# cmgcds/SParSH-AMG

Measured on AMD Instinct MI355X. Metric: AMG-PCG solve iterations/sec (7-pt 3D Poisson, fp64) + HBM GB/s (roofline: dominant kernel; config.whole_iteration: the iteration), higher is better.
Workload: dtype f64

## Files before the change

include/sparsh_amg.h:

```cpp
#ifndef SPARSH_AMG_H_
#define SPARSH_AMG_H_

#ifdef __cplusplus
extern "C" {
#endif

#define SPARSH_OK 0
#define SPARSH_EINVAL -1
#define SPARSH_ENODEV -2
#define SPARSH_ESTATE -3
#define SPARSH_ENUMERIC -4
#define SPARSH_ENOCONV -5
#define SPARSH_ECOMM -6

#define SPARSH_AMG 0
#define SPARSH_CG 1
#define SPARSH_PCG 2
#define SPARSH_BICG 3
#define SPARSH_PBICG 4
#define SPARSH_GMRES 5
#define SPARSH_PGMRES 6

#define SPARSH_SMOOTH_JACOBI 0
#define SPARSH_SMOOTH_SOR 1
#define SPARSH_SOR_FORWARD 0
#define SPARSH_SOR_SYMMETRIC 1

typedef struct sparsh_params {
    double omega;
    double tol;
    int sweeps;
    int max_levels;
    int limit_upper;
    int limit_lower;
    int coarsening;
    int max_iter;
    int coarse_limit;
    int host_threads;
    int device;
    int print_setup;
    int print_solve;
    int check_every;
    int use_graph;
    int replicate_rows;
    int precond_fp32;
    int dense_limit;
    int extend_until;
    int coarse_factor_mb;
} sparsh_params;

typedef struct sparsh_handle_s *sparsh_handle;

const char *sparsh_last_error(void);
int sparsh_version(void);
int sparsh_device_count(void);
int sparsh_host_cpus(void);

void sparsh_default_params(sparsh_params *p);

int sparsh_create_csr(int nrow, int ncol, const int *rowptr, const int *colindex, const double *val, sparsh_handle *out);
void sparsh_destroy(sparsh_handle h);

int sparsh_setup(sparsh_handle h, const sparsh_params *p);

int sparsh_set_stopping(sparsh_handle h, double tol, int max_iter, int check_every);

int sparsh_set_kernel_config(sparsh_handle h, int kind, int vec, int nt, int remap);

int sparsh_level_format(sparsh_handle h, int level, int *kind, long *stored_entries);

int sparsh_level_layout(sparsh_handle h, int level, long *slots, long *value_blocks, long *meta_bytes);
int sparsh_set_const_slots(sparsh_handle h, int enable);
int sparsh_set_index_compression(sparsh_handle h, int mode);
int sparsh_set_alternate_sweeps(sparsh_handle h, int mode);
int sparsh_set_paired_restriction(sparsh_handle h, int enable);
int sparsh_set_fused_prolongation(sparsh_handle h, int enable);
int sparsh_set_constant_diagonal(sparsh_handle h, int enable);
int sparsh_set_double_sweep(sparsh_handle h, int mode);
int sparsh_set_marching_ops(sparsh_handle h, int mode);
int sparsh_set_zero_start(sparsh_handle h, int enable);
int sparsh_set_deferred_x(sparsh_handle h, int enable);
int sparsh_level_marching_ops(sparsh_handle h, int level, int *on, int *plan, double *table_us, double *marching_us);
int sparsh_set_box_plan(sparsh_handle h, int level, int kernel, int q, int ty, int cz);
int sparsh_level_double_sweep(sparsh_handle h, int level, int *on, int *dims, int *plan, double *single_us, double *double_us);
int sparsh_level_constant_diagonal(sparsh_handle h, int level, int *is_const, double *value);
int sparsh_level_prolong_fused(sparsh_handle h, int level, int *fused);
int sparsh_level_paired(sparsh_handle h, int level, int *paired);
int sparsh_set_fused_zero_sweep(sparsh_handle h, int mode);
int sparsh_set_placement_search(sparsh_handle h, int enable);
int sparsh_placement_info(sparsh_handle h, double *chosen_us, double *worst_us, double *initial_us, int *triples, double *seconds);
int sparsh_set_setup_broadcast(sparsh_handle h, int enable);
int sparsh_setup_share_info(sparsh_handle h, int *built_locally, long *image_bytes);
long sparsh_debug_hierarchy_roundtrip(sparsh_handle h, long truncate_to);
int sparsh_level_index16(sparsh_handle h, int level, long *blocks16, long *blocks);
int sparsh_debug_index16_roundtrip(int nrow, const int *rowptr, const int *colindex, long *blocks16, long *blocks);
int sparsh_set_tile(sparsh_handle h, int enable);
int sparsh_level_tile_rows(sparsh_handle h, int level, int *rows);
int sparsh_bench_comm(sparsh_handle h, int what, int level, int reps, double *avg_seconds);
const char *sparsh_level_kernel(sparsh_handle h, int level);
int sparsh_level_placement(sparsh_handle h, int level, int *nt, int *remap);

int sparsh_setup_host(sparsh_handle h, const sparsh_params *p);

int sparsh_num_levels(sparsh_handle h);
int sparsh_level_info(sparsh_handle h, int level, int *nrow, int *nnz, int *p_ncol, int *p_nnz);
int sparsh_level_csr(sparsh_handle h, int level, int which, int *rowptr, int *colindex, double *val);
int sparsh_coarse_inverse(sparsh_handle h, double *inv);
int sparsh_coarse_info(sparsh_handle h, int *info6, long *bytes);
int sparsh_set_coarse_form(sparsh_handle h, int form, int leaf, int merge_rows);
int sparsh_set_coarse_top_merge(sparsh_handle h, int top_merge_rows);
int sparsh_coarse_nd_info(sparsh_handle h, int *info6);
int sparsh_coarse_window(sparsh_handle h, int *window);
int sparsh_set_coarse_interface(sparsh_handle h, int enable);
int sparsh_set_coarse_block(sparsh_handle h, int rows);
double sparsh_setup_seconds(sparsh_handle h);

int sparsh_vcycle(sparsh_handle h, const double *b, double *x, int iterations, double *hist, int hist_cap, int *ncycles);

int sparsh_vcycle_dev(sparsh_handle h, const double *b_dev, double *x_dev, int iterations, double *hist, int hist_cap, int *ncycles);

int sparsh_solve(sparsh_handle h, int method, const double *b, double *x, double *hist, int hist_cap, int *iters);

int sparsh_solve_dev(sparsh_handle h, int method, const double *b_dev, double *x_dev, int max_iters, double *hist, int hist_cap, int *iters, double *seconds);

int sparsh_krylov_init_dev(sparsh_handle h, int method, const double *b_dev, double *x_dev);
int sparsh_krylov_step_dev(sparsh_handle h, int nsteps, int *done, double *residual);
int sparsh_krylov_history(sparsh_handle h, double *hist, int hist_cap, int *iters);

int sparsh_op_spmv(sparsh_handle h, int level, const double *x, double *y);
int sparsh_op_jacobi(sparsh_handle h, int level, const double *b, double *x, int sweeps, int x_is_zero);
int sparsh_op_residual(sparsh_handle h, int level, const double *b, const double *x, double *r);
int sparsh_op_resnorm(sparsh_handle h, int level, const double *b, const double *x, double *nrm);
int sparsh_op_restrict(sparsh_handle h, int level, const double *r, double *bc);
int sparsh_op_residual_restrict(sparsh_handle h, int level, const double *b, const double *x, double *bc, double *xc);
int sparsh_op_prolong(sparsh_handle h, int level, const double *xc, double *xf);
int sparsh_op_jacobi_prolong(sparsh_handle h, int level, const double *b, const double *x, double *xf);
int sparsh_op_spmv_dot(sparsh_handle h, int level, const double *x, double *y, double *dot);
int sparsh_op_jacobi_dot(sparsh_handle h, int level, const double *b, const double *x, double *y, double *dot);
int sparsh_op_coarse(sparsh_handle h, const double *b, double *x);
int sparsh_op_precond_f32(sparsh_handle h, const double *r, double *z);
int sparsh_op_precond(sparsh_handle h, const double *r, double *z);
int sparsh_op_dot(sparsh_handle h, int n, const double *x, const double *y, double *out);
int sparsh_op_nrm2(sparsh_handle h, int n, const double *x, double *out);
int sparsh_op_axpby(sparsh_handle h, int n, double a, const double *x, double bcoef, double *y);

int sparsh_bench_op(sparsh_handle h, int op, int level, int reps, double *avg_seconds);

#define SPARSH_BASIS_FP64 0
#define SPARSH_BASIS_FP32 1
int sparsh_set_gmres(sparsh_handle h, int restart);
int sparsh_gmres_info(sparsh_handle h, int *restart, long *basis_bytes);
int sparsh_set_gmres_basis(sparsh_handle h, int precision);
int sparsh_gmres_basis(sparsh_handle h, int *precision);

int sparsh_set_smoother(sparsh_handle h, int kind, int sweeps, int order);
int sparsh_level_colors(sparsh_handle h, int level, int *ncolors, int *rows_per_color);
int sparsh_level_color_of_rows(sparsh_handle h, int level, int *color);
int sparsh_op_sor(sparsh_handle h, int level, const double *b, double *x, int sweeps, int reverse, int x_is_zero);
int sparsh_set_sor_path(sparsh_handle h, int mode);
int sparsh_level_sor_layout(sparsh_handle h, int level, int *ncolors, int *single_launch, long *bytes);

int sparsh_dev_alloc(sparsh_handle h, long nbytes, void **out);
int sparsh_dev_free(sparsh_handle h, void *p);
int sparsh_dev_fill(sparsh_handle h, double *dst_dev, long n, double value);
int sparsh_h2d(sparsh_handle h, void *dst_dev, const void *src, long nbytes);
int sparsh_d2h(sparsh_handle h, void *dst, const void *src_dev, long nbytes);
// ... 40 lines not shown
```

sparsh_amg_amd/__init__.py:

```python
from __future__ import annotations

import ctypes as C
import os

import numpy as np

from . import problems

_HERE = os.path.dirname(os.path.abspath(__file__))
LIB_PATH = os.path.join(_HERE, "libsparsh_amg.so")

SPARSH_AMG, SPARSH_CG, SPARSH_PCG, SPARSH_BICG, SPARSH_PBICG = 0, 1, 2, 3, 4
SPARSH_GMRES, SPARSH_PGMRES = 5, 6
METHODS = {"amg": SPARSH_AMG, "cg": SPARSH_CG, "pcg": SPARSH_PCG, "bicg": SPARSH_BICG, "pbicg": SPARSH_PBICG,
           "gmres": SPARSH_GMRES, "pgmres": SPARSH_PGMRES}
SPARSH_SMOOTH_JACOBI, SPARSH_SMOOTH_SOR = 0, 1
SPARSH_SOR_FORWARD, SPARSH_SOR_SYMMETRIC = 0, 1
SPARSH_BASIS_FP64, SPARSH_BASIS_FP32 = 0, 1
GMRES_BASES = {"fp64": SPARSH_BASIS_FP64, "fp32": SPARSH_BASIS_FP32}
SMOOTHERS = {"jacobi": SPARSH_SMOOTH_JACOBI, "sor": SPARSH_SMOOTH_SOR}
SOR_ORDERS = {"forward": SPARSH_SOR_FORWARD, "symmetric": SPARSH_SOR_SYMMETRIC}
SPARSH_OK, SPARSH_EINVAL, SPARSH_ENODEV, SPARSH_ESTATE, SPARSH_ENUMERIC, SPARSH_ENOCONV, SPARSH_ECOMM = 0, -1, -2, -3, -4, -5, -6

c_int_p = C.POINTER(C.c_int)
c_dbl_p = C.POINTER(C.c_double)


class SparshError(RuntimeError):
    def __init__(self, code, msg):
        super().__init__(f"sparsh error {code}: {msg}")
        self.code = code


class Params(C.Structure):

    _fields_ = [
        ("omega", C.c_double),
        ("tol", C.c_double),
        ("sweeps", C.c_int),
        ("max_levels", C.c_int),
        ("limit_upper", C.c_int),
        ("limit_lower", C.c_int),
        ("coarsening", C.c_int),
        ("max_iter", C.c_int),
        ("coarse_limit", C.c_int),
        ("host_threads", C.c_int),
        ("device", C.c_int),
        ("print_setup", C.c_int),
        ("print_solve", C.c_int),
        ("check_every", C.c_int),
        ("use_graph", C.c_int),
        ("replicate_rows", C.c_int),
        ("precond_fp32", C.c_int),
        ("dense_limit", C.c_int),
        ("extend_until", C.c_int),
        ("coarse_factor_mb", C.c_int),
    ]


def _load():
    if not os.path.exists(LIB_PATH):
        raise ImportError(
            f"{LIB_PATH} is missing: build it with `python -c 'import __graft_entry__ as g; g.build()'` "
            "(or `make -C sparsh_amg_amd/csrc`).  There is no pure-Python/CPU fallback."
        )
    L = C.CDLL(LIB_PATH)
    H = C.c_void_p
    P = C.POINTER
    sig = {
        "sparsh_last_error": (C.c_char_p, []),
        "sparsh_version": (C.c_int, []),
        "sparsh_device_count": (C.c_int, []),
        "sparsh_host_cpus": (C.c_int, []),
        "sparsh_default_params": (None, [P(Params)]),
        "sparsh_create_csr": (C.c_int, [C.c_int, C.c_int, c_int_p, c_int_p, c_dbl_p, P(H)]),
        "sparsh_destroy": (None, [H]),
        "sparsh_setup": (C.c_int, [H, P(Params)]),
        "sparsh_setup_host": (C.c_int, [H, P(Params)]),
        "sparsh_set_stopping": (C.c_int, [H, C.c_double, C.c_int, C.c_int]),
        "sparsh_set_kernel_config": (C.c_int, [H, C.c_int, C.c_int, C.c_int, C.c_int]),
        "sparsh_level_placement": (C.c_int, [H, C.c_int, c_int_p, c_int_p]),
        "sparsh_level_format": (C.c_int, [H, C.c_int, c_int_p, C.POINTER(C.c_long)]),
        "sparsh_level_layout": (C.c_int, [H, C.c_int, C.POINTER(C.c_long), C.POINTER(C.c_long), C.POINTER(C.c_long)]),
        "sparsh_set_const_slots": (C.c_int, [H, C.c_int]),
        "sparsh_set_tile": (C.c_int, [H, C.c_int]),
        "sparsh_set_index_compression": (C.c_int, [H, C.c_int]),
        "sparsh_set_alternate_sweeps": (C.c_int, [H, C.c_int]),
        "sparsh_set_paired_restriction": (C.c_int, [H, C.c_int]),
        "sparsh_set_fused_prolongation": (C.c_int, [H, C.c_int]),
        "sparsh_set_constant_diagonal": (C.c_int, [H, C.c_int]),
        "sparsh_set_double_sweep": (C.c_int, [H, C.c_int]),
        "sparsh_set_marching_ops": (C.c_int, [H, C.c_int]),
        "sparsh_set_zero_start": (C.c_int, [H, C.c_int]),
        "sparsh_set_deferred_x": (C.c_int, [H, C.c_int]),
        "sparsh_level_marching_ops": (C.c_int, [H, C.c_int, C.POINTER(C.c_int), C.POINTER(C.c_int), C.POINTER(C.c_double), C.POINTER(C.c_double)]),
        "sparsh_level_double_sweep": (C.c_int, [H, C.c_int, C.POINTER(C.c_int), C.POINTER(C.c_int), C.POINTER(C.c_int), C.POINTER(C.c_double),
                                                  C.POINTER(C.c_double)]),
        "sparsh_level_constant_diagonal": (C.c_int, [H, C.c_int, C.POINTER(C.c_int), C.POINTER(C.c_double)]),
        "sparsh_level_prolong_fused": (C.c_int, [H, C.c_int, C.POINTER(C.c_int)]),
        "sparsh_op_jacobi_prolong": (C.c_int, [H, C.c_int, c_dbl_p, c_dbl_p, c_dbl_p]),
        "sparsh_set_box_plan": (C.c_int, [H, C.c_int, C.c_int, C.c_int, C.c_int, C.c_int]),
        "sparsh_op_spmv_dot": (C.c_int, [H, C.c_int, c_dbl_p, c_dbl_p, c_dbl_p]),
        "sparsh_op_jacobi_dot": (C.c_int, [H, C.c_int, c_dbl_p, c_dbl_p, c_dbl_p, c_dbl_p]),
        "sparsh_level_paired": (C.c_int, [H, C.c_int, C.POINTER(C.c_int)]),
        "sparsh_set_fused_zero_sweep": (C.c_int, [H, C.c_int]),
        "sparsh_set_placement_search": (C.c_int, [H, C.c_int]),
        "sparsh_placement_info": (C.c_int, [H, C.POINTER(C.c_double), C.POINTER(C.c_double), C.POINTER(C.c_double), c_int_p, C.POINTER(C.c_double)]),
        "sparsh_debug_index16_roundtrip": (C.c_int, [C.c_int, c_int_p, c_int_p, C.POINTER(C.c_long), C.POINTER(C.c_long)]),
        "sparsh_set_setup_broadcast": (C.c_int, [H, C.c_int]),
        "sparsh_debug_hierarchy_roundtrip": (C.c_long, [H, C.c_long]),
        "sparsh_setup_share_info": (C.c_int, [H, C.POINTER(C.c_int), C.POINTER(C.c_long)]),
        "sparsh_level_index16": (C.c_int, [H, C.c_int, C.POINTER(C.c_long), C.POINTER(C.c_long)]),
        "sparsh_level_tile_rows": (C.c_int, [H, C.c_int, c_int_p]),
        "sparsh_bench_comm": (C.c_int, [H, C.c_int, C.c_int, C.c_int, c_dbl_p]),
        "sparsh_level_kernel": (C.c_char_p, [H, C.c_int]),
        "sparsh_num_levels": (C.c_int, [H]),
        "sparsh_level_info": (C.c_int, [H, C.c_int, c_int_p, c_int_p, c_int_p, c_int_p]),
        "sparsh_level_csr": (C.c_int, [H, C.c_int, C.c_int, c_int_p, c_int_p, c_dbl_p]),
        "sparsh_coarse_inverse": (C.c_int, [H, c_dbl_p]),
        "sparsh_op_precond_f32": (C.c_int, [H, c_dbl_p, c_dbl_p]),
        "sparsh_coarse_info": (C.c_int, [H, c_int_p, C.POINTER(C.c_long)]),
        "sparsh_coarse_window": (C.c_int, [H, c_int_p]),
        "sparsh_set_coarse_interface": (C.c_int, [H, C.c_int]),
        "sparsh_set_coarse_block": (C.c_int, [H, C.c_int]),
        "sparsh_set_coarse_form": (C.c_int, [H, C.c_int, C.c_int, C.c_int]),
        "sparsh_coarse_nd_info": (C.c_int, [H, c_int_p]),
        "sparsh_set_coarse_top_merge": (C.c_int, [H, C.c_int]),
        "sparsh_setup_seconds": (C.c_double, [H]),
        "sparsh_vcycle": (C.c_int, [H, c_dbl_p, c_dbl_p, C.c_int, c_dbl_p, C.c_int, c_int_p]),
        "sparsh_vcycle_dev": (C.c_int, [H, C.c_void_p, C.c_void_p, C.c_int, c_dbl_p, C.c_int, c_int_p]),
        "sparsh_solve": (C.c_int, [H, C.c_int, c_dbl_p, c_dbl_p, c_dbl_p, C.c_int, c_int_p]),
        "sparsh_solve_dev": (C.c_int, [H, C.c_int, C.c_void_p, C.c_void_p, C.c_int, c_dbl_p, C.c_int, c_int_p, c_dbl_p]),
        "sparsh_set_device": (C.c_int, [C.c_int]),
        "sparsh_comm_unique_id": (C.c_int, [C.c_char_p]),
        "sparsh_comm_init_rccl": (C.c_int, [H, C.c_char_p, C.c_int, C.c_int]),
        "sparsh_local_range": (C.c_int, [H, C.c_int, c_int_p, c_int_p, c_int_p]),
        "sparsh_set_overlap": (C.c_int, [H, C.c_int]),
        "sparsh_comm_group_create": (C.c_int, [C.c_int, P(C.c_void_p)]),
        "sparsh_comm_group_destroy": (None, [C.c_void_p]),
        "sparsh_set_deep_halo": (C.c_int, [H, C.c_int]),
        "sparsh_dist_deep_op": (C.c_int, [H, C.c_int, C.c_int, C.c_int, C.c_int, C.c_int, c_int_p]),
        "sparsh_dist_deep_op_get": (C.c_int, [H, c_int_p, c_int_p, c_dbl_p, c_int_p, c_int_p, c_int_p, c_int_p, c_int_p, c_int_p]),
        "sparsh_deep_info": (C.c_int, [H, C.c_int, c_int_p]),
        "sparsh_deep_layer_end": (C.c_int, [H, C.c_int, C.c_int, c_int_p]),
        "sparsh_deep_prefix_spmv": (C.c_int, [H, C.c_int, C.c_int, c_dbl_p, c_dbl_p]),
        "sparsh_exchanges_issued": (C.c_long, [H]),
        "sparsh_comm_group_fail_after": (C.c_int, [C.c_void_p, C.c_int]),
        "sparsh_comm_group_set_delay": (C.c_int, [C.c_void_p, C.c_double]),
        "sparsh_set_comm_tuning": (C.c_int, [H, C.c_int]),
        "sparsh_comm_schedule": (C.c_int, [H, C.c_int, c_int_p, c_dbl_p]),
        "sparsh_comm_measured": (C.c_int, [H, c_dbl_p]),
        "sparsh_plan_comm_schedule": (C.c_int, [H, C.c_int, c_dbl_p]),
        "sparsh_comm_init_group": (C.c_int, [H, C.c_void_p, C.c_int]),
        "sparsh_dist_local_op": (C.c_int, [H, C.c_int, C.c_int, C.c_int, C.c_int, c_int_p]),
        "sparsh_dist_local_op_get": (C.c_int, [H, c_int_p, c_int_p, c_dbl_p, c_int_p, c_int_p, c_int_p, c_int_p]),
        "sparsh_krylov_init_dev": (C.c_int, [H, C.c_int, C.c_void_p, C.c_void_p]),
        "sparsh_krylov_step_dev": (C.c_int, [H, C.c_int, c_int_p, c_dbl_p]),
        "sparsh_krylov_history": (C.c_int, [H, c_dbl_p, C.c_int, c_int_p]),
        "sparsh_op_spmv": (C.c_int, [H, C.c_int, c_dbl_p, c_dbl_p]),
        "sparsh_op_jacobi": (C.c_int, [H, C.c_int, c_dbl_p, c_dbl_p, C.c_int, C.c_int]),
        "sparsh_op_residual": (C.c_int, [H, C.c_int, c_dbl_p, c_dbl_p, c_dbl_p]),
        "sparsh_op_resnorm": (C.c_int, [H, C.c_int, c_dbl_p, c_dbl_p, c_dbl_p]),
        "sparsh_op_restrict": (C.c_int, [H, C.c_int, c_dbl_p, c_dbl_p]),
        "sparsh_op_residual_restrict": (C.c_int, [H, C.c_int, c_dbl_p, c_dbl_p, c_dbl_p, c_dbl_p]),
        "sparsh_op_prolong": (C.c_int, [H, C.c_int, c_dbl_p, c_dbl_p]),
        "sparsh_op_coarse": (C.c_int, [H, c_dbl_p, c_dbl_p]),
        "sparsh_op_dot": (C.c_int, [H, C.c_int, c_dbl_p, c_dbl_p, c_dbl_p]),
        "sparsh_op_nrm2": (C.c_int, [H, C.c_int, c_dbl_p, c_dbl_p]),
        "sparsh_op_axpby": (C.c_int, [H, C.c_int, C.c_double, c_dbl_p, C.c_double, c_dbl_p]),
        "sparsh_bench_op": (C.c_int, [H, C.c_int, C.c_int, C.c_int, c_dbl_p]),
        "sparsh_dev_alloc": (C.c_int, [H, C.c_long, P(C.c_void_p)]),
        "sparsh_dev_free": (C.c_int, [H, C.c_void_p]),
        "sparsh_dev_fill": (C.c_int, [H, C.c_void_p, C.c_long, C.c_double]),
        "sparsh_h2d": (C.c_int, [H, C.c_void_p, C.c_void_p, C.c_long]),
        "sparsh_d2h": (C.c_int, [H, C.c_void_p, C.c_void_p, C.c_long]),
        "sparsh_sync": (C.c_int, [H]),
        "sparsh_profile": (C.c_int, [H, C.c_int]),
        "sparsh_set_smoother": (C.c_int, [H, C.c_int, C.c_int, C.c_int]),
        "sparsh_level_colors": (C.c_int, [H, C.c_int, c_int_p, c_int_p]),
        "sparsh_level_color_of_rows": (C.c_int, [H, C.c_int, c_int_p]),
        "sparsh_op_sor": (C.c_int, [H, C.c_int, c_dbl_p, c_dbl_p, C.c_int, C.c_int, C.c_int]),
        "sparsh_set_sor_path": (C.c_int, [H, C.c_int]),
        "sparsh_level_sor_layout": (C.c_int, [H, C.c_int, c_int_p, c_int_p, C.POINTER(C.c_long)]),
        "sparsh_profile_read": (C.c_int, [H, c_dbl_p]),
        "sparsh_set_gmres": (C.c_int, [H, C.c_int]),
        "sparsh_gmres_info": (C.c_int, [H, c_int_p, C.POINTER(C.c_long)]),
        "sparsh_set_gmres_basis": (C.c_int, [H, C.c_int]),
        "sparsh_gmres_basis": (C.c_int, [H, c_int_p]),
        "sparsh_op_precond": (C.c_int, [H, c_dbl_p, c_dbl_p]),
    }
    for name, (res, args) in sig.items():
        fn = getattr(L, name)
        fn.restype = res
        fn.argtypes = args
    return L


lib = _load()


def _dp(a):
    return a.ctypes.data_as(c_dbl_p)


def _ip(a):
    return a.ctypes.data_as(c_int_p)


def _check(rc, allow=()):
    if rc != SPARSH_OK and rc not in allow:
        raise SparshError(rc, lib.sparsh_last_error().decode())
    return rc


def default_params(**kw) -> Params:
    p = Params()
    lib.sparsh_default_params(C.byref(p))
    for k, v in kw.items():
        if not hasattr(p, k):
            raise AttributeError(f"sparsh_params has no field {k}")
        setattr(p, k, v)
    return p


def set_device(device: int):
    _check(lib.sparsh_set_device(device))


def comm_unique_id() -> bytes:
    buf = C.create_string_buffer(128)
    _check(lib.sparsh_comm_unique_id(buf))
    return buf.raw


def comm_group_create(nranks: int):
    g = C.c_void_p()
    _check(lib.sparsh_comm_group_create(nranks, C.byref(g)))
    return g


def comm_group_destroy(g):
    lib.sparsh_comm_group_destroy(g)


def comm_group_set_delay(g, microseconds: float):
    _check(lib.sparsh_comm_group_set_delay(g, float(microseconds)))


def comm_group_fail_after(g, ncalls: int):
    _check(lib.sparsh_comm_group_fail_after(g, int(ncalls)))


def index16_roundtrip(rowptr, colindex):
    rp = np.ascontiguousarray(rowptr, dtype=np.int32)
    ci = np.ascontiguousarray(colindex, dtype=np.int32)
    a, b = C.c_long(), C.c_long()
    _check(lib.sparsh_debug_index16_roundtrip(len(rp) - 1, _ip(rp), _ip(ci), C.byref(a), C.byref(b)))
    return a.value, b.value


def device_count() -> int:
    return lib.sparsh_device_count()


def host_cpus() -> int:
    return lib.sparsh_host_cpus()


class sp_matrix_mg:

    def __init__(self, rowptr, colindex, val, ncol=None):
        self.rowptr = np.ascontiguousarray(rowptr, dtype=np.int32)
        self.colindex = np.ascontiguousarray(colindex, dtype=np.int32)
        self.val = np.ascontiguousarray(val, dtype=np.float64)
        self.nrow = len(self.rowptr) - 1
        self.ncol = self.nrow if ncol is None else int(ncol)
        self.nnz = int(self.rowptr[-1])
        if len(self.colindex) < self.nnz or len(self.val) < self.nnz:
            raise ValueError("colindex/val shorter than rowptr[-1]")
        h = C.c_void_p()
        _check(lib.sparsh_create_csr(self.nrow, self.ncol, _ip(self.rowptr), _ip(self.colindex), _dp(self.val), C.byref(h)))
        self._h = h
        self.params = None

    def close(self):
        if getattr(self, "_h", None):
            lib.sparsh_destroy(self._h)
            self._h = None

    def __del__(self):
        try:
            self.close()
        except Exception:
            pass

    def set_const_slots(self, enable=True):
        _check(lib.sparsh_set_const_slots(self._h, int(bool(enable))))
        return self

    def set_setup_broadcast(self, enable=True):
        _check(lib.sparsh_set_setup_broadcast(self._h, int(bool(enable))))
        return self

    def hierarchy_roundtrip(self, truncate_to=-1):
        r = lib.sparsh_debug_hierarchy_roundtrip(self._h, int(truncate_to))
        if r < 0:
            _check(int(r))
        return int(r)

    def setup_share_info(self):
        a, b = C.c_int(), C.c_long()
        _check(lib.sparsh_setup_share_info(self._h, C.byref(a), C.byref(b)))
        return bool(a.value), b.value

    def set_placement_search(self, enable=True):
        _check(lib.sparsh_set_placement_search(self._h, int(bool(enable))))
        return self

    def placement_info(self):
        a, b, c, k, t = C.c_double(), C.c_double(), C.c_double(), C.c_int(), C.c_double()
        _check(lib.sparsh_placement_info(self._h, C.byref(a), C.byref(b), C.byref(c), C.byref(k), C.byref(t)))
        return {"chosen_us": round(a.value, 2), "worst_us": round(b.value, 2), "initial_us": round(c.value, 2), "triples": k.value,
                "seconds": round(t.value, 3)}

    def set_fused_zero_sweep(self, enable=2):
        _check(lib.sparsh_set_fused_zero_sweep(self._h, int(enable)))
        return self

    def set_alternate_sweeps(self, mode=1):
        _check(lib.sparsh_set_alternate_sweeps(self._h, int(mode)))
        return self

    def set_double_sweep(self, mode=1):
        _check(lib.sparsh_set_double_sweep(self._h, int(mode)))
        return self

    def level_double_sweep(self, level):
        on = C.c_int(0)
        dims, plan = (C.c_int * 3)(), (C.c_int * 3)()
        t1, t2 = C.c_double(0.0), C.c_double(0.0)
        _check(lib.sparsh_level_double_sweep(self._h, int(level), C.byref(on), dims, plan, C.byref(t1), C.byref(t2)))
        return {"on": bool(on.value), "grid": list(dims), "points_per_thread": plan[0], "lines_per_tile": plan[1], "planes_per_chunk": plan[2],
                "two_single_sweeps_us": round(t1.value, 2), "double_sweep_us": round(t2.value, 2)}

    def set_deferred_x(self, enable=True):
        _check(lib.sparsh_set_deferred_x(self._h, 1 if enable else 0))
        return self

    def set_zero_start(self, enable=True):
        _check(lib.sparsh_set_zero_start(self._h, 1 if enable else 0))
        return self

    def set_marching_ops(self, mode=1):
        _check(lib.sparsh_set_marching_ops(self._h, int(mode)))
        return self

    def level_marching_ops(self, level):
        on = C.c_int(0)
        plan = (C.c_int * 3)()
        t1, t2 = C.c_double(0.0), C.c_double(0.0)
        _check(lib.sparsh_level_marching_ops(self._h, int(level), C.byref(on), plan, C.byref(t1), C.byref(t2)))
        return {"on": bool(on.value), "points_per_thread": plan[0], "lines_per_tile": plan[1], "planes_per_chunk": plan[2],
                "table_kernel_us": round(t1.value, 2), "marching_kernel_us": round(t2.value, 2)}

    def set_box_plan(self, level, kernel, q=0, ty=0, cz=0, shared_cu=False):
        k = {"double": 2, "marching": 1}.get(kernel, kernel)
        if shared_cu:
            if k != 1:
                raise ValueError("shared_cu is a plan of the marching kernel")
            k = 3
        _check(lib.sparsh_set_box_plan(self._h, int(level), int(k), int(q), int(ty), int(cz)))
        return self

    def set_constant_diagonal(self, enable=True):
        _check(lib.sparsh_set_constant_diagonal(self._h, 1 if enable else 0))
        return self

    def level_constant_diagonal(self, level):
        f, v = C.c_int(0), C.c_double(0.0)
        _check(lib.sparsh_level_constant_diagonal(self._h, int(level), C.byref(f), C.byref(v)))
        return bool(f.value), v.value

    def set_fused_prolongation(self, enable=True):
        _check(lib.sparsh_set_fused_prolongation(self._h, 1 if enable else 0))
        return self

    def level_prolong_fused(self, level):
        v = C.c_int(0)
        _check(lib.sparsh_level_prolong_fused(self._h, int(level), C.byref(v)))
        return v.value

    def op_jacobi_prolong(self, level, b, x, xf):
        b = np.ascontiguousarray(b, dtype=np.float64)
        x = np.ascontiguousarray(x, dtype=np.float64)
        xf = np.array(xf, dtype=np.float64)
        _check(lib.sparsh_op_jacobi_prolong(self._h, int(level), _dp(b), _dp(x), _dp(xf)))
        return xf

    def set_paired_restriction(self, enable=True):
        _check(lib.sparsh_set_paired_restriction(self._h, 1 if enable else 0))
        return self

    def level_paired(self, level):
        v = C.c_int(0)
        _check(lib.sparsh_level_paired(self._h, int(level), C.byref(v)))
        return v.value

    def set_index_compression(self, mode=1):
        _check(lib.sparsh_set_index_compression(self._h, int(mode)))
        return self

    def level_index16(self, level):
        a, b = C.c_long(), C.c_long()
        _check(lib.sparsh_level_index16(self._h, level, C.byref(a), C.byref(b)))
        return a.value, b.value

    def set_tile(self, enable=True):
        _check(lib.sparsh_set_tile(self._h, int(bool(enable))))
        return self

    def level_tile_rows(self, level):
        r = C.c_int(0)
        _check(lib.sparsh_level_tile_rows(self._h, level, C.byref(r)))
        return r.value

    def set_smoother(self, kind="jacobi", sweeps=0, order="forward"):
        k = SMOOTHERS[kind] if isinstance(kind, str) else int(kind)
        o = SOR_ORDERS[order] if isinstance(order, str) else int(order)
        _check(lib.sparsh_set_smoother(self._h, k, int(sweeps), o))
        return self

    def set_gmres(self, restart=0, basis=None):
        _check(lib.sparsh_set_gmres(self._h, int(restart)))
        if basis is not None:
            _check(lib.sparsh_set_gmres_basis(self._h, GMRES_BASES[basis] if isinstance(basis, str) else int(basis)))
        return self

    def gmres_basis(self):
        p = C.c_int()
        _check(lib.sparsh_gmres_basis(self._h, C.byref(p)))
        return {v: k for k, v in GMRES_BASES.items()}[p.value]

    def gmres_info(self):
        m, nbytes = C.c_int(), C.c_long()
        _check(lib.sparsh_gmres_info(self._h, C.byref(m), C.byref(nbytes)))
        info = dict(restart=m.value, basis_bytes=nbytes.value)
        if self.gmres_basis() != "fp64":
            info["basis"] = self.gmres_basis()
        return info

    def level_colors(self, level):
        nc = C.c_int(0)
        _check(lib.sparsh_level_colors(self._h, level, C.byref(nc), None))
        counts = np.zeros(max(nc.value, 1), dtype=np.int32)
        _check(lib.sparsh_level_colors(self._h, level, C.byref(nc), _ip(counts)))
# ... 215 lines not shown
        _check(lib.sparsh_dist_deep_op_get(self._h, _ip(rp), _ip(ci), _dp(v), _ip(gof), _ip(le), _ip(si), _ip(ss), _ip(rpos), _ip(rs)))
        M = sp.csr_matrix((v[:nnz], ci[:nnz], rp), shape=(nrow, nall))
        recv = rs[: 3 * nrs].reshape(-1, 3)
        nrecv = int(recv[:, 2].sum()) if len(recv) else 0
        plan = dict(nloc=nloc, npad=npad, nall=nall, global_of=gof[:nall], layer_end=le, send_idx=si[:nsend],
                    send=ss[: 3 * nss].reshape(-1, 3), recv=recv, recv_pos=rpos[:nrecv])
        return M, plan

    def vcycle(self, b, x, iterations=-1, hist_cap=8192):
        b = np.ascontiguousarray(b, dtype=np.float64)
        hist = np.zeros(hist_cap)
        n = C.c_int()
        rc = _check(lib.sparsh_vcycle(self._h, _dp(b), _dp(x), iterations, _dp(hist), hist_cap, C.byref(n)), allow=(SPARSH_ENOCONV,))
        return hist[: min(n.value, hist_cap)].copy(), rc

    def solve(self, method, b, x, hist_cap=8192, allow=()):
        b = np.ascontiguousarray(b, dtype=np.float64)
        assert x.dtype == np.float64 and x.flags.c_contiguous
        hist = np.zeros(hist_cap)
        n = C.c_int()
        m = METHODS[method] if isinstance(method, str) else method
        rc = _check(lib.sparsh_solve(self._h, m, _dp(b), _dp(x), _dp(hist), hist_cap, C.byref(n)), allow=(SPARSH_ENOCONV,) + tuple(allow))
        return hist[: min(n.value, hist_cap)].copy(), rc

    def dev_alloc(self, nbytes):
        p = C.c_void_p()
        _check(lib.sparsh_dev_alloc(self._h, nbytes, C.byref(p)))
        return p

    def dev_free(self, p):
        _check(lib.sparsh_dev_free(self._h, p))

    def dev_fill(self, dptr, n, value=0.0):
        _check(lib.sparsh_dev_fill(self._h, dptr, n, value))

    def h2d(self, dptr, arr):
        arr = np.ascontiguousarray(arr)
        _check(lib.sparsh_h2d(self._h, dptr, arr.ctypes.data_as(C.c_void_p), arr.nbytes))

    def d2h(self, arr, dptr):
        _check(lib.sparsh_d2h(self._h, arr.ctypes.data_as(C.c_void_p), dptr, arr.nbytes))

    def sync(self):
        _check(lib.sparsh_sync(self._h))

    def solve_dev(self, method, b_dev, x_dev, max_iters=0, hist_cap=8192):
        hist = np.zeros(hist_cap)
        n = C.c_int()
        sec = C.c_double()
        m = METHODS[method] if isinstance(method, str) else method
        rc = _check(
            lib.sparsh_solve_dev(self._h, m, b_dev, x_dev, max_iters, _dp(hist), hist_cap, C.byref(n), C.byref(sec)),
            allow=(SPARSH_ENOCONV,),
        )
        return hist[: min(n.value, hist_cap)].copy(), n.value, sec.value, rc

    def krylov_init_dev(self, method, b_dev, x_dev):
        m = METHODS[method] if isinstance(method, str) else method
        _check(lib.sparsh_krylov_init_dev(self._h, m, b_dev, x_dev))

    def krylov_step_dev(self, nsteps):
        done = C.c_int()
        res = C.c_double()
        _check(lib.sparsh_krylov_step_dev(self._h, nsteps, C.byref(done), C.byref(res)))
        return done.value, res.value

    def krylov_history(self, hist_cap=8192):
        hist = np.zeros(hist_cap)
        n = C.c_int()
        _check(lib.sparsh_krylov_history(self._h, _dp(hist), hist_cap, C.byref(n)))
        return hist[: min(n.value, hist_cap)].copy()

    def profile(self, enable=True):
        _check(lib.sparsh_profile(self._h, 1 if enable else 0))

    def profile_read(self):
        out = np.zeros(4)
        _check(lib.sparsh_profile_read(self._h, _dp(out)))
        return dict(launches=int(out[0]), seconds=out[1], nrow=int(out[2]), nnz=int(out[3]))

    def bench_op(self, op, level=0, reps=20):
        ops = {"spmv": 0, "jacobi": 1, "residual": 2, "restrict": 3, "prolong": 4, "coarse": 5, "dot": 6, "axpby": 7, "copy_int": 8,
               "jacobi_pingpong": 9, "jacobi_pingpong_resident": 10, "jacobi_double": 11, "sor": 12,
               "gmres_orth": 13, "gmres_orth_unfused": 14, "gmres_orth_fp32_basis": 15}
        sec = C.c_double()
        _check(lib.sparsh_bench_op(self._h, ops[op] if isinstance(op, str) else op, level, reps, C.byref(sec)))
        return sec.value

    def op_spmv(self, level, x):
        x = np.ascontiguousarray(x, dtype=np.float64)
        y = np.zeros(self.level_info(level)["nrow"])
        _check(lib.sparsh_op_spmv(self._h, level, _dp(x), _dp(y)))
        return y

    def op_jacobi(self, level, b, x, sweeps, x_is_zero=False):
        b = np.ascontiguousarray(b, dtype=np.float64)
        x = np.array(x, dtype=np.float64)
        _check(lib.sparsh_op_jacobi(self._h, level, _dp(b), _dp(x), sweeps, 1 if x_is_zero else 0))
        return x

    def op_sor(self, level, b, x, sweeps, reverse=False, x_is_zero=False):
        b = np.ascontiguousarray(b, dtype=np.float64)
        x = np.array(x, dtype=np.float64)
        _check(lib.sparsh_op_sor(self._h, level, _dp(b), _dp(x), int(sweeps), 1 if reverse else 0, 1 if x_is_zero else 0))
        return x

    def op_residual(self, level, b, x):
        b = np.ascontiguousarray(b, dtype=np.float64)
        x = np.ascontiguousarray(x, dtype=np.float64)
        r = np.zeros_like(b)
        _check(lib.sparsh_op_residual(self._h, level, _dp(b), _dp(x), _dp(r)))
        return r

    def op_resnorm(self, level, b, x):
        b = np.ascontiguousarray(b, dtype=np.float64)
        x = np.ascontiguousarray(x, dtype=np.float64)
        out = C.c_double()
        _check(lib.sparsh_op_resnorm(self._h, level, _dp(b), _dp(x), C.byref(out)))
        return out.value

    def op_spmv_dot(self, level, x):
        x = np.ascontiguousarray(x, dtype=np.float64)
        y = np.zeros(self.level_info(level)["nrow"])
        dot = C.c_double()
        _check(lib.sparsh_op_spmv_dot(self._h, int(level), _dp(x), _dp(y), C.byref(dot)))
        return y, dot.value

    def op_jacobi_dot(self, level, b, x):
        b = np.ascontiguousarray(b, dtype=np.float64)
        x = np.ascontiguousarray(x, dtype=np.float64)
        y = np.zeros_like(b)
        dot = C.c_double()
        _check(lib.sparsh_op_jacobi_dot(self._h, int(level), _dp(b), _dp(x), _dp(y), C.byref(dot)))
        return y, dot.value

    def op_restrict(self, level, r):
        r = np.ascontiguousarray(r, dtype=np.float64)
        bc = np.zeros(self.level_info(level + 1)["nrow"])
        _check(lib.sparsh_op_restrict(self._h, level, _dp(r), _dp(bc)))
        return bc

    def op_residual_restrict(self, level, b, x):
        b = np.ascontiguousarray(b, dtype=np.float64)
        x = np.ascontiguousarray(x, dtype=np.float64)
        nc = self.level_info(level + 1)["nrow"]
        bc, xc = np.zeros(nc), np.zeros(nc)
        _check(lib.sparsh_op_residual_restrict(self._h, level, _dp(b), _dp(x), _dp(bc), _dp(xc)))
        return bc, xc

    def op_prolong(self, level, xc, xf):
        xc = np.ascontiguousarray(xc, dtype=np.float64)
        xf = np.array(xf, dtype=np.float64)
        _check(lib.sparsh_op_prolong(self._h, level, _dp(xc), _dp(xf)))
        return xf

    def op_coarse(self, b):
        b = np.ascontiguousarray(b, dtype=np.float64)
        x = np.zeros_like(b)
        _check(lib.sparsh_op_coarse(self._h, _dp(b), _dp(x)))
        return x

    def op_precond_f32(self, r):
        r = np.ascontiguousarray(r, dtype=np.float64)
        z = np.zeros_like(r)
        _check(lib.sparsh_op_precond_f32(self._h, _dp(r), _dp(z)))
        return z

# ... 65 lines not shown
```

sparsh_amg_amd/csrc/capi.cpp:

```cpp
#include <algorithm>
#include <cmath>
#include <cstdio>
#include <cstdlib>
#include <cstring>
#include <memory>
#include <string>
#include <vector>

#include <hip/hip_runtime_api.h>

#include "../../include/sparsh_amg.h"
#include "engine.hpp"

using namespace sparsh;

struct sparsh_handle_s {
    std::unique_ptr<Engine> eng;
    LocalOp cached_op;
    DeepLocal cached_deep;
};

namespace {

thread_local std::string g_err;
// ... 370 lines not shown
    return SPARSH_OK;
}

int sparsh_set_alternate_sweeps(sparsh_handle h, int enable)
{
    if (!h || !h->eng) return fail(SPARSH_EINVAL, "null handle");
    if (enable < 0 || enable > 2) return fail(SPARSH_EINVAL, "mode must be 0 (never), 1 (where a sweep streams more than the Infinity Cache holds) or 2 (always)");
    h->eng->kernel_cfg().alt_dir = enable;
    h->eng->config_changed();
    return SPARSH_OK;
}

int sparsh_set_double_sweep(sparsh_handle h, int mode)
{
    if (!h || !h->eng) return fail(SPARSH_EINVAL, "null handle");
    if (mode < 0 || mode > 2) return fail(SPARSH_EINVAL, "mode must be 0 (never), 1 (where the setup measures it faster) or 2 (wherever the level is a box grid with a plan)");
    h->eng->kernel_cfg().box2 = mode;
    h->eng->config_changed();
    return SPARSH_OK;
}

int sparsh_level_double_sweep(sparsh_handle h, int level, int *on, int *dims, int *plan, double *single_us, double *double_us)
{
    REQUIRE_READY(h);
    REQUIRE_LEVEL(h, level);
    const DevLevel &L = h->eng->level(level);
    if (on) *on = (!h->eng->distributed() || L.replicated) && box2_applies(L.A, h->eng->kernel_cfg()) ? 1 : 0;
    if (dims) {
        dims[0] = L.A.box_nx;
        dims[1] = L.A.box_ny;
        dims[2] = L.A.box_nz;
    }
    if (plan) {
        plan[0] = L.A.box_q;
        plan[1] = L.A.box_ty;
        plan[2] = L.A.box_cz;
    }
    if (single_us) *single_us = L.box_single_us;
    if (double_us) *double_us = L.box_double_us;
    return SPARSH_OK;
}

int sparsh_set_deferred_x(sparsh_handle h, int enable)
{
    if (!h || !h->eng) return fail(SPARSH_EINVAL, "null handle");
    h->eng->kernel_cfg().defer_x = enable != 0;
    h->eng->config_changed();
    return SPARSH_OK;
}

int sparsh_set_zero_start(sparsh_handle h, int enable)
{
    if (!h || !h->eng) return fail(SPARSH_EINVAL, "null handle");
    h->eng->kernel_cfg().zero_start = enable != 0;
    h->eng->config_changed();
    return SPARSH_OK;
}

int sparsh_set_marching_ops(sparsh_handle h, int mode)
{
    if (!h || !h->eng) return fail(SPARSH_EINVAL, "null handle");
    if (mode < 0 || mode > 2) return fail(SPARSH_EINVAL, "mode must be 0 (never), 1 (where the setup measures it faster) or 2 (wherever the level is a box grid with a plan)");
    h->eng->kernel_cfg().box1 = mode;
    h->eng->config_changed();
    return SPARSH_OK;
}

int sparsh_level_marching_ops(sparsh_handle h, int level, int *on, int *plan, double *table_us, double *marching_us)
{
    REQUIRE_READY(h);
    REQUIRE_LEVEL(h, level);
    const DevLevel &L = h->eng->level(level);
    if (on) *on = (!h->eng->distributed() || L.replicated) && box1_applies(L.A, h->eng->kernel_cfg()) ? 1 : 0;
    if (plan) {
        plan[0] = L.A.box1_q;
        plan[1] = L.A.box1_ty;
        plan[2] = L.A.box1_cz;
    }
    if (table_us) *table_us = L.box1_table_us;
    if (marching_us) *marching_us = L.box1_us;
    return SPARSH_OK;
}

int sparsh_set_box_plan(sparsh_handle h, int level, int kernel, int q, int ty, int cz)
{
    REQUIRE_READY(h);
    REQUIRE_LEVEL(h, level);
    const int rc = h->eng->set_box_plan(level, kernel, q, ty, cz);
    return rc == SPARSH_OK ? SPARSH_OK : fail(rc, h->eng->error);
}

int sparsh_set_constant_diagonal(sparsh_handle h, int enable)
{
    if (!h || !h->eng) return fail(SPARSH_EINVAL, "null handle");
    h->eng->kernel_cfg().const_diag = enable != 0;
    h->eng->config_changed();
    return SPARSH_OK;
}

int sparsh_level_constant_diagonal(sparsh_handle h, int level, int *is_const, double *value)
{
    REQUIRE_READY(h);
    REQUIRE_LEVEL(h, level);
    const DevLevel &L = h->eng->level(level);
    if (is_const) *is_const = h->eng->diag_stream(L) == nullptr ? 1 : 0;
    if (value) *value = L.diag_const;
    return SPARSH_OK;
}

int sparsh_set_fused_prolongation(sparsh_handle h, int enable)
{
    if (!h || !h->eng) return fail(SPARSH_EINVAL, "null handle");
    h->eng->kernel_cfg().fuse_prolong = enable != 0;
    h->eng->config_changed();
    return SPARSH_OK;
}

int sparsh_level_prolong_fused(sparsh_handle h, int level, int *fused)
{
    REQUIRE_READY(h);
    REQUIRE_LEVEL(h, level);
    if (!fused) return fail(SPARSH_EINVAL, "null output");
    *fused = !h->eng->level_prolong_fused(level) ? 0 : (h->eng->level(level - 1).pair_aggregates ? 1 : 2);
    return SPARSH_OK;
}

int sparsh_set_paired_restriction(sparsh_handle h, int enable)
{
    if (!h || !h->eng) return fail(SPARSH_EINVAL, "null handle");
    h->eng->kernel_cfg().pair_restrict = enable != 0;
    h->eng->config_changed();
    return SPARSH_OK;
}

int sparsh_level_paired(sparsh_handle h, int level, int *paired)
{
    REQUIRE_READY(h);
    REQUIRE_LEVEL(h, level);
    if (!paired) return fail(SPARSH_EINVAL, "null output");
    *paired = h->eng->level_paired(level);
    return SPARSH_OK;
}

int sparsh_set_index_compression(sparsh_handle h, int mode)
{
    if (!h || !h->eng) return fail(SPARSH_EINVAL, "null handle");
    if (mode < 0 || mode > 2) return fail(SPARSH_EINVAL, "mode must be 0 (off), 1 (operators that stream from HBM through the CSR-stream kernel) or 2 (every operator)");
    h->eng->kernel_cfg().idx16 = mode;
    h->eng->config_changed();
    return SPARSH_OK;
}

int sparsh_level_index16(sparsh_handle h, int level, long *blocks16, long *blocks)
{
    REQUIRE_READY(h);
    REQUIRE_LEVEL(h, level);
    const DevCsr &A = h->eng->level(level).A;
    if (blocks16) *blocks16 = A.col16 ? A.nblk16 : 0;
    if (blocks) *blocks = A.nblk;
    return SPARSH_OK;
}

int sparsh_set_smoother(sparsh_handle h, int kind, int sweeps, int order)
{
    if (!h || !h->eng) return fail(SPARSH_EINVAL, "null handle");
    Engine &E = *h->eng;
    if (kind != SPARSH_SMOOTH_JACOBI && kind != SPARSH_SMOOTH_SOR)
        return fail(SPARSH_EINVAL, "kind must be SPARSH_SMOOTH_JACOBI (0) or SPARSH_SMOOTH_SOR (1)");
    if (sweeps < 0) return fail(SPARSH_EINVAL, "sweeps < 0");
    if (order != SPARSH_SOR_FORWARD && order != SPARSH_SOR_SYMMETRIC)
        return fail(SPARSH_EINVAL, "order must be SPARSH_SOR_FORWARD (0) or SPARSH_SOR_SYMMETRIC (1)");
    if (kind == SPARSH_SMOOTH_JACOBI && sweeps > 0 && E.ready() && E.distributed())
// ... 744 lines not shown
}

int sparsh_op_nrm2(sparsh_handle h, int n, const double *x, double *out)
{
    double d = 0.0;
    int rc = sparsh_op_dot(h, n, x, x, &d);
    if (rc == SPARSH_OK) *out = std::sqrt(d);
    return rc;
}

int sparsh_op_axpby(sparsh_handle h, int n, double a, const double *x, double bcoef, double *y)
{
    REQUIRE_READY(h);
    REQUIRE_SINGLE(h);
    if (n <= 0) return fail(SPARSH_EINVAL, "n <= 0");
    Engine &E = *h->eng;
    DBuf dx(E, (size_t)n, x), dy(E, (size_t)n, y);
    launch_axpby(n, a, dx.p, bcoef, dy.p, E.stream());
    return done(E, dy.get(y));
}

int sparsh_bench_op(sparsh_handle h, int op, int level, int reps, double *avg_seconds)
{
    REQUIRE_READY(h);
    REQUIRE_LEVEL(h, level);
    if (reps <= 0 || !avg_seconds) return fail(SPARSH_EINVAL, "bad reps");
    Engine &E = *h->eng;
    const DevLevel &L = E.level(level);
    const size_t n = (size_t)L.n;
    const bool has_coarse = level + 1 < E.nlevels();
    if ((op == 3 || op == 4) && !has_coarse) return fail(SPARSH_EINVAL, "no coarser level");
    const size_t nc = has_coarse ? (size_t)E.level(level + 1).n : 1;
    const size_t xh = (size_t)std::max(L.planA.nhalo, L.planR.nhalo), ch = (size_t)L.planP.nhalo;
    DBuf x(E, n + xh), y(E, n), b(E, n), c(E, nc + ch);
    std::vector<double> ones(std::max(n, nc), 1.0);
    (void)hipMemcpy(x.p, ones.data(), n * 8, hipMemcpyHostToDevice);
    (void)hipMemcpy(b.p, ones.data(), n * 8, hipMemcpyHostToDevice);
    (void)hipMemcpy(y.p, ones.data(), n * 8, hipMemcpyHostToDevice);
    (void)hipMemcpy(c.p, ones.data(), nc * 8, hipMemcpyHostToDevice);
    hipStream_t st = E.stream();
    auto run = [&]() {
        switch (op) {
        case 0: E.op_spmv(level, x.p, y.p); break;
        case 1: {
            CsrArgs a;
            a.x = x.p;
            a.b = b.p;
            a.d = L.diag;
            a.y = y.p;
            a.omega = E.params().omega;
            launch_csr(L.A, OP_JACOBI, a, L.fine, st, E.kernel_cfg());
        } break;
        case 2: E.op_residual(level, b.p, x.p, y.p); break;
        case 3: E.op_restrict(level, x.p, c.p); break;
        case 4: E.op_prolong(level, c.p, y.p); break;
        case 5: E.op_coarse(E.level(E.nlevels() - 1).b ? E.level(E.nlevels() - 1).b : b.p, E.level(E.nlevels() - 1).r); break;
        case 6: {
            int nb = 0;
            launch_dot((int)n, x.p, b.p, E.level(0).r, &nb, st);
        } break;
        case 7: launch_axpby((int)n, 0.5, x.p, 0.5, y.p, st); break;
        case 8: launch_copy_int((int)n, L.A.rowptr, reinterpret_cast<int *>(y.p), st); break;
        case 9:
        case 10: {
            static thread_local int flip = 0;
            double *xa = op == 9 ? x.p : L.x, *xb = op == 9 ? y.p : L.x2;
            CsrArgs a;
            a.x = (flip & 1) ? xb : xa;
            a.y = (flip & 1) ? xa : xb;
            a.b = op == 9 ? b.p : L.r;
            a.d = L.diag;
            a.omega = E.params().omega;
            a.reverse = csr_alternates(L.A, E.kernel_cfg()) && (flip & 1);
            ++flip;
            launch_csr(L.A, OP_JACOBI, a, L.fine, st, E.kernel_cfg());
        } break;
        case 12: E.sor_leg(level, L.r, L.x, 1, false); break;
        case 11: {
            static thread_local int flip2 = 0;
            double *xa = (flip2 & 1) ? L.x2 : L.x, *xb = (flip2 & 1) ? L.x : L.x2;
            ++flip2;
            launch_box2(L.A, xa, L.r, xb, E.params().omega, L.fine, st);
        } break;
        case 13: E.gmres_bench_step(true); break;
        case 14: E.gmres_bench_step(false); break;
        case 15: E.gmres_bench_step(true); break;
        default: break;
        }
    };
    if (op < 0 || op > 15) return fail(SPARSH_EINVAL, "unknown op");
    if (op == 13 || op == 14 || op == 15) {
        if (level != 0 || E.distributed()) return fail(SPARSH_EINVAL, "the GMRES orthogonalisation step runs on level 0 of a single-GPU handle");
        if ((op == 15) != (E.gmres_basis() == SPARSH_BASIS_FP32))
            return fail(SPARSH_ESTATE, "ops 13 and 14 run on a double basis, op 15 on a float basis (sparsh_set_gmres_basis)");
        if (int rc = E.gmres_bench_prepare(); rc != SPARSH_OK) return fail(rc, E.error);
    }
    if (op == 12 && (E.distributed() || !E.build_sor_level(level))) return fail(SPARSH_ESTATE, "no SOR layout on this handle");
    if (op == 11 && (E.distributed() || !box2_applies(L.A, E.kernel_cfg()))) return fail(SPARSH_ESTATE, "the level does not run double sweeps (sparsh_level_double_sweep)");
    for (int i = 0; i < 3; ++i) run();
    hipEvent_t e0, e1;
    (void)hipEventCreate(&e0);
    (void)hipEventCreate(&e1);
    (void)hipEventRecord(e0, st);
    for (int i = 0; i < reps; ++i) run();
    (void)hipEventRecord(e1, st);
    (void)hipEventSynchronize(e1);
    float ms = 0.f;
    (void)hipEventElapsedTime(&ms, e0, e1);
    (void)hipEventDestroy(e0);
    (void)hipEventDestroy(e1);
    *avg_seconds = ms * 1e-3 / reps;
    return SPARSH_OK;
}

int sparsh_dev_alloc(sparsh_handle h, long nbytes, void **out)
{
    if (!h || !h->eng || !out || nbytes < 0) return fail(SPARSH_EINVAL, "bad arguments");
    *out = h->eng->dalloc((size_t)nbytes);
    return *out ? SPARSH_OK : fail(SPARSH_ENODEV, h->eng->error);
}

int sparsh_dev_free(sparsh_handle h, void *p)
{
    if (!h || !h->eng) return fail(SPARSH_EINVAL, "null handle");
    h->eng->dfree(p);
    return SPARSH_OK;
}

int sparsh_dev_fill(sparsh_handle h, double *dst_dev, long n, double value)
{
    if (!h || !h->eng || !h->eng->stream()) return fail(SPARSH_EINVAL, "null handle or no stream (call sparsh_setup first)");
    if (n < 0 || n > 0x7fffffffL) return fail(SPARSH_EINVAL, "bad length");
    launch_fill((int)n, value, dst_dev, h->eng->stream());
    return SPARSH_OK;
}

int sparsh_h2d(sparsh_handle h, void *dst_dev, const void *src, long nbytes)
{
    if (!h || !h->eng) return fail(SPARSH_EINVAL, "null handle");
    if (hipMemcpy(dst_dev, src, (size_t)nbytes, hipMemcpyHostToDevice) != hipSuccess) return fail(SPARSH_ENODEV, "H2D failed");
    return SPARSH_OK;
}

int sparsh_d2h(sparsh_handle h, void *dst, const void *src_dev, long nbytes)
{
    if (!h || !h->eng) return fail(SPARSH_EINVAL, "null handle");
    if (h->eng->stream()) (void)hipStreamSynchronize(h->eng->stream());
    if (hipMemcpy(dst, src_dev, (size_t)nbytes, hipMemcpyDeviceToHost) != hipSuccess) return fail(SPARSH_ENODEV, "D2H failed");
    return SPARSH_OK;
}

int sparsh_sync(sparsh_handle h)
{
    if (!h || !h->eng) return fail(SPARSH_EINVAL, "null handle");
    if (h->eng->stream() && hipStreamSynchronize(h->eng->stream()) != hipSuccess) return fail(SPARSH_ENODEV, "sync failed");
    return SPARSH_OK;
}

int sparsh_profile(sparsh_handle h, int enable)
{
    if (!h || !h->eng) return fail(SPARSH_EINVAL, "null handle");
    if (enable) {
        h->eng->profile_begin();
        h->eng->prof.enabled = true;
    } else if (h->eng->prof.enabled) {
        h->eng->profile_collect();
        h->eng->prof.enabled = false;
    }
    return SPARSH_OK;
}

int sparsh_profile_read(sparsh_handle h, double *out4)
{
    REQUIRE_READY(h);
    out4[0] = h->eng->prof.launches;
    out4[1] = h->eng->prof.seconds;
    out4[2] = h->eng->level(0).n;
    out4[3] = h->eng->level(0).A.nnz;
    return SPARSH_OK;
}

}
```

sparsh_amg_amd/csrc/engine.cpp:

```cpp
#include "engine.hpp"

#include <algorithm>
#include <functional>
#include <cmath>
#include <cstdio>
#include <cstdlib>
#include <cstring>
#include <omp.h>

namespace sparsh {

namespace {
constexpr int kProfEvents = 8192;
}

bool Engine::check(hipError_t e, const char *what)
{
    if (e == hipSuccess) return true;
    error = std::string(what) + ": " + hipGetErrorString(e);
    return false;
}

bool Engine::note_hip(hipError_t e, const char *what)
{
// ... 485 lines not shown
    const double t0 = omp_get_wtime();
    omp_set_num_threads(p.host_threads > 0 ? p.host_threads : effective_cpus());
    std::vector<char> image;
    int rc0 = SPARSH_OK;
    std::string err0;
    if (me == 0) {
        rc0 = setup_host(p);
        err0 = error;
        if (rc0 == SPARSH_OK) serialize_hierarchy(H_, image);
    }
    built_locally_ = (me == 0);
    long long *hdr = nullptr;
    if (!check(hipMalloc(reinterpret_cast<void **>(&hdr), 16), "hipMalloc")) return SPARSH_ENODEV;
    long long h2[2] = {(long long)image.size(), (long long)rc0};
    bool good = check(hipMemcpyAsync(hdr, h2, 16, hipMemcpyHostToDevice, st_), "hipMemcpy");
    good = good && comm_->bcast(hdr, 16, 0, st_);
    good = good && check(hipMemcpyAsync(h2, hdr, 16, hipMemcpyDeviceToHost, st_), "hipMemcpy") && check(hipStreamSynchronize(st_), "hipStreamSynchronize");
    (void)hipFree(hdr);
    if (!good) {
        if (error.empty()) error = "broadcast of the hierarchy header failed: " + comm_->error;
        return SPARSH_ECOMM;
    }
    if (h2[1] != SPARSH_OK) {
        error = me == 0 ? err0 : "the setup on rank 0 failed";
        host_ready_ = false;
        return (int)h2[1];
    }
    const size_t total = (size_t)h2[0];
    image_bytes_ = total;
    if (me != 0) image.resize(total);
    const size_t chunk = std::min<size_t>(total, (size_t)256 << 20);
    char *stage = nullptr;
    {
        const bool mine = chunk == 0 || hipMalloc(reinterpret_cast<void **>(&stage), chunk) == hipSuccess;
        double *flag = nullptr;
        if (!check(hipMalloc(reinterpret_cast<void **>(&flag), sizeof(double)), "hipMalloc")) {
            if (stage) (void)hipFree(stage);
            return SPARSH_ENODEV;
        }
        double f = mine ? 0.0 : 1.0;
        bool okf = check(hipMemcpyAsync(flag, &f, sizeof(double), hipMemcpyHostToDevice, st_), "hipMemcpy") && comm_->allreduce_sum(flag, 1, st_) &&
                   check(hipMemcpyAsync(&f, flag, sizeof(double), hipMemcpyDeviceToHost, st_), "hipMemcpy") && check(hipStreamSynchronize(st_), "hipStreamSynchronize");
        (void)hipFree(flag);
        if (!okf || f != 0.0) {
            if (stage) (void)hipFree(stage);
            if (!okf) {
                if (error.empty()) error = "agreement on the hierarchy staging buffers failed: " + comm_->error;
                return SPARSH_ECOMM;
            }
            error = mine ? "another rank could not allocate its staging buffer for the hierarchy broadcast"
                         : "hipMalloc of the " + std::to_string(chunk >> 20) + " MB staging buffer for the hierarchy broadcast failed";
            return SPARSH_ENODEV;
        }
    }
    for (size_t off = 0; good && off < total; off += chunk) {
        const size_t nb = std::min(chunk, total - off);
        if (me == 0) good = check(hipMemcpyAsync(stage, image.data() + off, nb, hipMemcpyHostToDevice, st_), "hipMemcpy");
        good = good && comm_->bcast(stage, nb, 0, st_);
        if (good && me != 0) good = check(hipMemcpyAsync(image.data() + off, stage, nb, hipMemcpyDeviceToHost, st_), "hipMemcpy");
        good = good && check(hipStreamSynchronize(st_), "hipStreamSynchronize");
    }
    if (stage) (void)hipFree(stage);
    if (!good) {
        if (error.empty()) error = "broadcast of the hierarchy failed: " + comm_->error;
        return SPARSH_ECOMM;
    }
    if (me != 0) {
        prm_ = p;
        ready_ = false;
        if (!deserialize_hierarchy(image.data(), image.size(), A0_, H_)) {
            error = H_.error;
            host_ready_ = false;
            return SPARSH_ENUMERIC;
        }
        host_ready_ = true;
        setup_seconds = omp_get_wtime() - t0;
        H_.seconds = setup_seconds;
    }
    return SPARSH_OK;
}

void Engine::tune_box_kernels()
{
    for (size_t l = 0; l + 1 < lev_.size(); ++l) {
        DevLevel &L = lev_[l];
        L.A.box_on = L.A.box1_on = false;
        L.box_single_us = L.box_double_us = L.box1_table_us = L.box1_us = 0.0;
        if (L.A.box_q <= 0 || (dist_ && !L.replicated) || L.deep || csr_family(L.A, cfg_) != FAM_SDIA_TAB) continue;
        if (cfg_.box2 >= 2) L.A.box_on = true;
        if (cfg_.box1 >= 2) L.A.box1_on = L.A.box1_q > 0;
        const bool time2 = cfg_.box2 == 1, time1 = cfg_.box1 == 1 && L.A.box1_q > 0;
        if (!(time1 || time2)) continue;
        if (L.n < 400000) continue;
        hipEvent_t e0 = nullptr, e1 = nullptr;
        if (hipEventCreate(&e0) != hipSuccess || hipEventCreate(&e1) != hipSuccess) continue;
        CsrArgs a;
        a.b = L.r;
        launch_fill(L.n, 1.0, L.r, st_);
        a.d = L.diag;
        a.omega = prm_.omega;
        auto timed = [&](bool fused) -> double {
            double *p = L.x, *q = L.x2;
            const int launches = fused ? 5 : 10;
            for (int it = 0; it < launches; ++it) {
                if (it == (fused ? 1 : 2)) (void)hipEventRecord(e0, st_);
                if (fused) {
                    launch_box2(L.A, p, a.b, q, prm_.omega, L.fine, st_);
                } else {
                    a.x = p;
                    a.y = q;
                    launch_csr(L.A, OP_JACOBI, a, L.fine, st_, cfg_);
                }
                std::swap(p, q);
            }
            (void)hipEventRecord(e1, st_);
            if (hipEventSynchronize(e1) != hipSuccess) return 1e30;
            float ms = 0.f;
            (void)hipEventElapsedTime(&ms, e0, e1);
            return (double)ms * 1e3 / 4.0;
        };
        if (time2) {
            L.box_single_us = timed(false);
            L.box_double_us = timed(true);
            L.A.box_on = L.box_double_us < 0.97 * L.box_single_us;
        }
        if (time1) {
            auto timed1 = [&](bool marching) -> double {
                double *p = L.x, *q = L.x2;
                for (int it = 0; it < 8; ++it) {
                    if (it == 2) (void)hipEventRecord(e0, st_);
                    a.x = p;
                    a.y = q;
                    a.partial = part0_;
                    if (marching) launch_box1(L.A, 1, a, L.fine, st_);
                    else launch_csr(L.A, OP_JACOBI_DOT, a, L.fine, st_, cfg_);
                    std::swap(p, q);
                }
                (void)hipEventRecord(e1, st_);
                if (hipEventSynchronize(e1) != hipSuccess) return 1e30;
                float ms = 0.f;
                (void)hipEventElapsedTime(&ms, e0, e1);
                return (double)ms * 1e3 / 6.0;
            };
            L.box1_table_us = timed1(false);
            L.box1_us = timed1(true);
            {
                const int q0 = L.A.box1_q, ty0 = L.A.box1_ty, cz0 = L.A.box1_cz;
                if (box1_plan(L.A, true) && (L.A.box1_q != q0 || L.A.box1_ty != ty0 || L.A.box1_cz != cz0) && box1_workgroups(L.A) <= part_cap_) {
                    const double t_alt = timed1(true);
                    if (t_alt < L.box1_us) {
                        L.box1_us = t_alt;
                    } else {
                        L.A.box1_q = q0;
                        L.A.box1_ty = ty0;
                        L.A.box1_cz = cz0;
                    }
                } else {
                    L.A.box1_q = q0;
                    L.A.box1_ty = ty0;
                    L.A.box1_cz = cz0;
                }
            }
            L.A.box1_on = L.box1_us < 0.97 * L.box1_table_us;
        }
        (void)hipMemsetAsync(L.x, 0, (size_t)L.n * 8, st_);
        (void)hipMemsetAsync(L.x2, 0, (size_t)L.n * 8, st_);
        (void)hipMemsetAsync(L.r, 0, (size_t)L.n * 8, st_);
        (void)hipEventDestroy(e0);
        (void)hipEventDestroy(e1);
    }
}

void Engine::tune_placement()
{
    if (lev_.size() < 2) return;
    DevLevel &L = lev_[0];
    const size_t bytes = (size_t)L.n * 24;
    if (bytes < ((size_t)96 << 20) || bytes > ((size_t)512 << 20)) return;
    const CsrFamily fam = csr_family(L.A, cfg_);
    if (fam != FAM_SDIA_TAB) return;
    std::vector<double **> slots = {&L.x, &L.x2, &work_[0], &L.r};
    for (size_t k = 1; k < work_.size(); ++k) slots.push_back(&work_[k]);
    std::vector<double *> buf;
    for (double **s : slots) buf.push_back(*s);
    const size_t owned = buf.size();
    const size_t vbytes = (size_t)L.n * 8;
    for (int q = 0; q < 5; ++q) {
        void *sp = nullptr;
        if (hipMalloc(&sp, vbytes) != hipSuccess) break;
        buf.push_back(static_cast<double *>(sp));
    }
    hipEvent_t e0 = nullptr, e1 = nullptr;
    if (hipEventCreate(&e0) != hipSuccess || hipEventCreate(&e1) != hipSuccess) {
        for (size_t q = owned; q < buf.size(); ++q) (void)hipFree(buf[q]);
        return;
    }
    auto probe = [&](double *x, double *x2, double *b) -> double {
        CsrArgs a;
        a.b = b;
        a.d = L.diag;
        a.omega = prm_.omega;
        double *p = x, *q = x2;
        const bool pairs = box2_applies(L.A, cfg_);
        for (int it = 0; it < (pairs ? 5 : 10); ++it) {
            if (it == (pairs ? 1 : 2)) (void)hipEventRecord(e0, st_);
            if (pairs) {
                launch_box2(L.A, p, b, q, prm_.omega, L.fine, st_);
            } else {
                a.x = p;
                a.y = q;
                launch_csr(L.A, OP_JACOBI, a, L.fine, st_, cfg_);
            }
            std::swap(p, q);
        }
        (void)hipEventRecord(e1, st_);
        if (hipEventSynchronize(e1) != hipSuccess) return 1e30;
        float ms = 0.f;
        (void)hipEventElapsedTime(&ms, e0, e1);
        return (double)ms * 1e3 / 8.0;
    };
    const double t_begin = omp_get_wtime();
    for (double *q : buf) launch_fill(L.n, 1.0, q, st_);
    const double good_us = (double)L.n * 24.0 / 5.8e12 * 1e6 * 1.04 * (box2_applies(L.A, cfg_) ? 0.6 : 1.0);
    double best = 1e30, worst = 0.0;
    int bi = 0, bj = 1, bk = 2;
    const int nb = (int)buf.size();
    bool done = false;
    for (int hi = 2; hi < nb && !done; ++hi)
        for (int j = 1; j < hi && !done; ++j)
            for (int i = 0; i < j && !done; ++i) {
                const double t = probe(buf[i], buf[j], buf[hi]);
                if (place_tried == 0) place_first_us = t;
                ++place_tried;
                if (t < best) {
                    best = t;
                    bi = i;
                    bj = j;
                    bk = hi;
                }
                worst = std::max(worst, t);
                done = best <= good_us || place_tried >= 260;
            }
    (void)hipEventDestroy(e0);
    (void)hipEventDestroy(e1);
// ... 480 lines not shown
            const Partition &rrows = parts_[l + 1].replicated ? gather_part_ : parts_[l + 1];
            LocalOp lr = extract_local(h.R, rrows, pl, me);
            if (!upload_csr(*this, lp.M, d.P, false) || !upload_plan(lp.plan, d.planP)) return SPARSH_ENODEV;
            if (!upload_csr(*this, lr.M, d.R, false) || !upload_plan(lr.plan, d.planR)) return SPARSH_ENODEV;
            d.P_is_aggregation = h.P_is_aggregation;
            int xh = d.planA.nhalo;
            if (l > 0 && !lev_[l - 1].replicated) xh = std::max(xh, lev_[l - 1].planP.nhalo);
            xcap = (size_t)d.n + xh;
            rcap = (size_t)d.n + d.planR.nhalo;
            if (d.deep) {
                xcap = (size_t)d.layer_end[d.K];
                rcap = std::max((size_t)d.npad, (size_t)d.n + d.planR.nhalo) + 64;
                d.xc_stage = static_cast<double *>(dalloc(((size_t)d.planP.nloc + d.planP.nhalo + 64) * 8));
                if (!d.xc_stage) return SPARSH_ENODEV;
                if (l == 0) {
                    d.b_ext = static_cast<double *>(dalloc(xcap * 8));
                    if (!d.b_ext || !check(hipMemsetAsync(d.b_ext, 0, xcap * 8, st_), "hipMemsetAsync")) return SPARSH_ENODEV;
                }
            }
        }
        d.x = static_cast<double *>(dalloc(xcap * 8));
        d.x2 = static_cast<double *>(dalloc(xcap * 8));
        d.r = static_cast<double *>(dalloc(rcap * 8));
        if (l > 0) {
            const size_t bcap = d.deep ? xcap : (size_t)d.n;
            d.b = static_cast<double *>(dalloc(bcap * 8));
            if (d.b && !check(hipMemsetAsync(d.b, 0, bcap * 8, st_), "hipMemsetAsync")) return SPARSH_ENODEV;
        }
        if (!d.diag || !d.x || !d.x2 || !d.r || (l > 0 && !d.b)) return SPARSH_ENODEV;
        if (l + 1 < nl) max_blk = std::max(max_blk, std::max(partial_count(d.P), partial_count(d.R)));
        max_blk = std::max(max_blk, partial_count(d.A));
        if (!check(hipMemsetAsync(d.x, 0, xcap * 8, st_), "hipMemsetAsync")) return SPARSH_ENODEV;
        if (!check(hipMemsetAsync(d.x2, 0, xcap * 8, st_), "hipMemsetAsync")) return SPARSH_ENODEV;
        if (!check(hipMemsetAsync(d.r, 0, rcap * 8, st_), "hipMemsetAsync")) return SPARSH_ENODEV;
    }
    phase("last level: layouts + uploads");
    nL_ = H_.nL;
    if (H_.coarse_dense) {
        if (!coarse_.setup_dense(nL_, H_.coarse_inverse.data(), error)) return SPARSH_ENODEV;
        std::vector<double>().swap(H_.coarse_inverse);
    } else {
        const double t_f = omp_get_wtime();
        int why = 0;
        const bool okc = coarse_.form() == 1 ? coarse_.setup_bt(H_.levels.back().A, st_, error, &why) : coarse_.setup_nd(H_.levels.back().A, st_, error, &why);
        if (!okc) return why == 1 ? SPARSH_EINVAL : (why == 2 ? SPARSH_ENUMERIC : SPARSH_ENODEV);
        setup_seconds += omp_get_wtime() - t_f;
        if (p.print_setup && (G == 1 || me == 0)) {
            if (coarse_.nested())
                std::printf("coarsest level: %d rows, nested dissection: %d nodes on %d levels (largest pivot block %d), factors %.1f MB in HBM, %d launches per solve, %.2f s\n",
                            nL_, coarse_.nd().nnodes(), coarse_.nd().nlevels(), coarse_.nd().max_pivot_rows(), coarse_.bytes() / 1e6,
                            coarse_.nd().launches_per_solve(), coarse_.factor_seconds);
            else
                std::printf("coarsest level: %d rows, RCM bandwidth %d -> %d blocks of %d, factors %.1f MB in HBM, %.2f s\n", nL_, coarse_.bandwidth(),
                            coarse_.nblocks(), coarse_.block(), coarse_.bytes() / 1e6, coarse_.factor_seconds);
        }
    }

    part_cap_ = max_blk + 8;
    part0_ = static_cast<double *>(dalloc((size_t)part_cap_ * 8));
    part1_ = static_cast<double *>(dalloc((size_t)part_cap_ * 8));
    scal_ = static_cast<double *>(dalloc(S_COUNT * 8));
    hist_cap_dev_ = std::max(1024, p.max_iter + 2);
    hist_cap_dev_ = std::min(hist_cap_dev_, 1 << 22);
    hist_dev_ = static_cast<double *>(dalloc((size_t)hist_cap_dev_ * 8));
    iter_ctr_ = static_cast<int *>(dalloc(sizeof(int)));
    if (!part0_ || !part1_ || !scal_ || !hist_dev_ || !iter_ctr_) return SPARSH_ENODEV;
    if (!check(hipMemsetAsync(scal_, 0, S_COUNT * 8, st_), "hipMemsetAsync")) return SPARSH_ENODEV;
    if (!check(hipMemsetAsync(iter_ctr_, 0, sizeof(int), st_), "hipMemsetAsync")) return SPARSH_ENODEV;
    drop_graph();
    if (!pinned_ && !check(hipHostMalloc(reinterpret_cast<void **>(&pinned_), 64 * sizeof(double), hipHostMallocDefault), "hipHostMalloc"))
        return SPARSH_ENODEV;
    work_.clear();
    const size_t wcap = lev_[0].deep ? (size_t)lev_[0].layer_end[lev_[0].K] : (size_t)lev_[0].n + lev_[0].planA.nhalo;
    for (int k = 0; k < 8; ++k) {
        double *w = static_cast<double *>(dalloc(wcap * 8));
        if (!w) return SPARSH_ENODEV;
        if (!check(hipMemsetAsync(w, 0, wcap * 8, st_), "hipMemsetAsync")) return SPARSH_ENODEV;
        work_.push_back(w);
    }
    place_tried = 0;
    place_best_us = place_worst_us = place_first_us = 0.0;
    phase("coarsest-level factorisation + workspace");
    tune_box_kernels();
    if (G == 1 && cfg_.place_search) tune_placement();
    phase("placement search");
    f32_ready_ = false;
    if (p.precond_fp32 && !setup_f32()) return SPARSH_EINVAL;
    if (dist_ && !st2_) {
        if (!check(hipStreamCreateWithFlags(&st2_, hipStreamNonBlocking), "hipStreamCreate") ||
            !check(hipEventCreateWithFlags(&ev_ready_, hipEventDisableTiming), "hipEventCreate") ||
            !check(hipEventCreateWithFlags(&ev_halo_, hipEventDisableTiming), "hipEventCreate"))
            return SPARSH_ENODEV;
    }
    if (sor_on() && !dist_ && !p.precond_fp32 && !build_sor_layouts()) return SPARSH_ENODEV;
    if (!check(hipStreamSynchronize(st_), "setup sync")) return SPARSH_ENODEV;
    if (!comm_->barrier(st_)) {
        error = "comm barrier after setup failed: " + comm_->error;
        return SPARSH_ECOMM;
    }
    ready_ = true;
    return SPARSH_OK;
}

bool Engine::setup_f32()
{
    const int nl = (int)lev_.size();
    if (dist_) {
        error = "precond_fp32 is implemented for one GPU";
        return false;
    }
    if (nl < 2) return true;
    f32_.assign((size_t)nl, F32Level());
    for (int l = 0; l < nl; ++l) {
        DevLevel &d = lev_[l];
        F32Level &f = f32_[l];
        const size_t n = (size_t)d.n;
        f.x = static_cast<float *>(dalloc(n * 4));
        f.b = static_cast<float *>(dalloc(n * 4));
        if (!f.x || !f.b) return false;
        if (l + 1 < nl) {
            f.x2 = static_cast<float *>(dalloc(n * 4));
            f.r = static_cast<float *>(dalloc(n * 4));
            f.diag = static_cast<float *>(dalloc(n * 4));
            if (!f.x2 || !f.r || !f.diag) return false;
            launch_cvt_d2f((long)n, d.diag, f.diag, st_);
            if (d.A.has_sdia()) {
                f.A.nrow = d.n;
                f.A.nslice = d.A.nslice;
                f.A.sd_ptr = d.A.sd_ptr;
                f.A.sd_off = d.A.sd_off;
                f.A.sd_mask = d.A.sd_mask;
                f.A.slots = d.A.sd_slots;
                f.A.val = static_cast<float *>(dalloc((size_t)d.A.sd_slots * 64 * 4));
                if (!f.A.val) return false;
                launch_cvt_d2f((long)d.A.sd_slots * 64, d.A.sd_val, f.A.val, st_);
            } else {
                f.csr_val = static_cast<float *>(dalloc((size_t)std::max(d.A.nnz, 1) * 4));
                if (!f.csr_val) return false;
                launch_cvt_d2f((long)d.A.nnz, d.A.val, f.csr_val, st_);
            }
        }
    }
    if (coarse_.dense()) {
        coarse_inv_f32_ = static_cast<float *>(dalloc((size_t)nL_ * nL_ * 4));
        if (!coarse_inv_f32_) return false;
        launch_cvt_d2f((long)nL_ * nL_, coarse_.dense_inverse(), coarse_inv_f32_, st_);
    } else {
        coarse_inv_f32_ = nullptr;
        coarse_tmp_ = static_cast<double *>(dalloc((size_t)nL_ * 2 * 8));
        if (!coarse_tmp_) return false;
    }
    f32_ready_ = true;
    return true;
}

void Engine::vcycle_f32(const double *r64, double *z64, double *partial, int *nblk)
{
    const int last = (int)lev_.size() - 1;
    const int nu = prm_.sweeps;
    const float w = (float)prm_.omega;
    launch_cvt_d2f((long)lev_[0].n, r64, f32_[0].b, st_);
    auto apply = [&](int l, CsrOp op, const float *x, float *y) {
        F32Level &f = f32_[l];
        if (f.A.val)
            launch_sdia_f32(f.A, op, x, f.b, y, w, st_);
        else
// ... 135 lines not shown
    launch_finalize(code, p0, p1, nblk, scal_, slot, hist, it, st_, 1, iter_ctr_, hist_cap_dev_, nblk1);
    note_comm(comm_->allreduce_sum(scal_ + S_SUM0, 2, st_), "allreduce");
    launch_finalize(code, p0, p1, nblk, scal_, slot, hist, it, st_, 2, iter_ctr_, hist_cap_dev_, nblk1);
}


void Engine::op_spmv(int l, const double *x, double *y)
{
    CsrArgs a;
    a.x = x;
    a.y = y;
    apply_A(lev_[l], OP_SPMV, a);
}

void Engine::op_residual(int l, const double *b, const double *x, double *r)
{
    CsrArgs a;
    a.x = x;
    a.b = b;
    a.y = r;
    apply_A(lev_[l], OP_RESID, a);
}

void Engine::op_residual_restrict(int l, const double *b, const double *x, double *bc, double *xc)
{
    if (!lev_[l].pair_aggregates && lev_[l].pair_axis != 0) {
        launch_box_resid_pair(lev_[l].A, lev_[l].pair_axis, x, b, diag_stream(lev_[l + 1]), lev_[l + 1].diag_const, prm_.omega, bc, xc, st_);
        return;
    }
    CsrArgs a;
    a.x = x;
    a.b = b;
    a.y = bc;
    a.y2 = xc;
    a.d = diag_stream(lev_[l + 1]);
    a.dconst = lev_[l + 1].diag_const;
    a.omega = prm_.omega;
    if (box1_applies(lev_[l].A, cfg_) && lev_[l].A.box_nx % 2 == 0) {
        launch_box1(lev_[l].A, 2, a, lev_[l].fine, st_);
        return;
    }
    launch_resid_pair(lev_[l].A, a, lev_[l].fine, st_, cfg_);
}

void Engine::op_jacobi_prolong(int l, const double *b, const double *x, double *xf)
{
    DevLevel &F = lev_[l - 1];
    CsrArgs a;
    a.x = x;
    a.b = b;
    a.d = lev_[l].diag;
    a.omega = prm_.omega;
    a.y2 = xf;
    a.members = F.pair_aggregates ? nullptr : F.members;
    a.nfine = F.n;
    apply_A(lev_[l], OP_JACOBI_PROLONG, a);
}

double Engine::op_spmv_dot(int l, const double *x, double *y)
{
    CsrArgs a;
    a.x = x;
    a.y = y;
    a.partial = part0_;
    const int np = apply_A(lev_[l], OP_SPMV_DOT, a);
    finalize(FIN_STORE, part0_, nullptr, np, S_TMP, nullptr, 0);
    return read_scalar(S_TMP);
}

double Engine::op_jacobi_dot(int l, const double *b, const double *x, double *y)
{
    CsrArgs a;
    a.x = x;
    a.b = b;
    a.y = y;
    a.d = lev_[l].diag;
    a.omega = prm_.omega;
    a.partial = part0_;
    const int np = apply_A(lev_[l], OP_JACOBI_DOT, a);
    finalize(FIN_STORE, part0_, nullptr, np, S_TMP, nullptr, 0);
    return read_scalar(S_TMP);
}

int Engine::set_box_plan(int l, int kernel, int q, int ty, int cz)
{
    auto refuse = [&](const std::string &why) {
        error = why;
        return SPARSH_EINVAL;
    };
    DevCsr &A = lev_[l].A;
    if (A.box_nx <= 0) return refuse("level " + std::to_string(l) + " is not a box grid");
    if (kernel < 1 || kernel > 3) return refuse("kernel must be 2 (double sweep), 1 (plane-marching kernel) or 3 (its shared-CU plan)");
    const bool planner = q == 0 && ty == 0 && cz == 0;
    if (kernel == 3 && !planner) return refuse("kernel 3 takes the planner's shared-CU plan: q, ty and cz must be 0");
    DevCsr T = A;
    if (planner) {
        if (!(kernel == 2 ? box2_plan(T) : box1_plan(T, kernel == 3))) return refuse("the planner has no plan for this grid");
        q = kernel == 2 ? T.box_q : T.box1_q;
        ty = kernel == 2 ? T.box_ty : T.box1_ty;
        cz = kernel == 2 ? T.box_cz : T.box1_cz;
    }
    if (const char *why = box_plan_refusal(A, kernel == 2 ? 2 : 1, q, ty, cz)) return refuse(why);
    if (kernel == 2) {
        A.box_q = q;
        A.box_ty = ty;
        A.box_cz = cz;
    } else {
        T.box1_q = q;
        T.box1_ty = ty;
        T.box1_cz = cz;
        if (box1_workgroups(T) > part_cap_)
            return refuse("the plan launches " + std::to_string(box1_workgroups(T)) + " workgroups; the partial buffers hold " + std::to_string(part_cap_));
        A.box1_q = q;
        A.box1_ty = ty;
        A.box1_cz = cz;
    }
    config_changed();
    return SPARSH_OK;
}

double Engine::op_resnorm(int l, const double *b, const double *x)
{
    CsrArgs a;
    a.x = x;
    a.b = b;
    a.partial = part0_;
    const int np = apply_A(lev_[l], OP_RESNORM, a);
    finalize(FIN_SQRT, part0_, nullptr, np, S_RES, nullptr, 0);
    return read_scalar(S_RES);
}

bool Engine::op_restrict(int l, const double *r, double *bc, bool fuse_zero)
{
    DevLevel &L = lev_[l];
    halo(L.planR, const_cast<double *>(r));
    CsrArgs a;
    a.x = r;
    const bool gather = dist_ && !L.replicated && lev_[l + 1].replicated;
    a.y = gather ? bc + gather_part_.lo(comm_->rank) : bc;
    bool fused = false;
    if (L.P_is_aggregation && fuse_zero && !gather && l + 2 < (int)lev_.size() && lev_[l + 1].n == L.R.nrow) {
        launch_restrict_agg_zero(L.R.nrow, L.R.rowptr, L.R.col, r, a.y, diag_stream(lev_[l + 1]), lev_[l + 1].diag_const, prm_.omega, lev_[l + 1].x, st_);
        fused = true;
    } else if (L.P_is_aggregation) {
        launch_restrict_agg(L.R.nrow, L.R.rowptr, L.R.col, r, a.y, st_);
    } else {
        launch_csr(L.R, OP_SPMV, a, false, st_, cfg_);
    }
    if (gather) note_comm(comm_->allgather(bc, gather_part_, st_), "allgather");
    return fused;
}

void Engine::op_prolong(int l, const double *xc, double *xf)
{
    DevLevel &L = lev_[l];
    if (L.deep && !lev_[l + 1].replicated) {
        launch_copy(L.planP.nloc, xc, L.xc_stage, st_);
        xc = L.xc_stage;
    }
    halo(L.planP, const_cast<double *>(xc));
    if (L.P_is_aggregation) {
        launch_prolong_agg(L.n, L.P.col, xc, xf, st_);
    } else {
        CsrArgs a;
        a.x = xc;
        a.y = xf;
        launch_csr(L.P, OP_ADD, a, false, st_, cfg_);
    }
}

void Engine::op_coarse(const double *b, double *x) { coarse_.solve(b, x, st_); }

double Engine::op_dot(int n, const double *x, const double *y)
{
    int nb = 0;
    launch_dot(n, x, y, part0_, &nb, st_);
    finalize(FIN_STORE, part0_, nullptr, nb, S_TMP, nullptr, 0);
    return read_scalar(S_TMP);
}

void Engine::smooth(DevLevel &L, const double *b, int sweeps, bool x_zero, double *dot_partial, int *dot_nblk, bool zero_done,
                    DevLevel *prolong_to)
{
    if (L.deep) {
        const int K = L.K;
        int s = 0;
        const bool timed = prof.enabled && &L == &lev_[0] && prof.used + 2 <= prof.ev.size();
        int in_run = 0;
        if (x_zero && sweeps > 0) {
            if (!zero_done) launch_jacobi_zero(L.layer_end[K - 1], b, L.diag, 0.0, prm_.omega, L.x, st_);
            s = 1;
        }
        if (timed) HIPCHK(hipEventRecord(prof.ev[prof.used], st_));
        for (; s < sweeps; ++s) {
            CsrArgs a;
// ... 917 lines not shown
```

sparsh_amg_amd/csrc/engine.hpp:

```cpp
#pragma once

#include <memory>
#include <string>
#include <vector>

#include "../../include/sparsh_amg.h"
#include "coarse.hpp"
#include "comm.hpp"
#include "dist.hpp"
#include "host_setup.hpp"
#include "kernels.hpp"

namespace sparsh {

struct DevLevel {
    bool deep = false;
    int K = 0;
    int npad = 0;
    std::vector<int> layer_end;
    DevDeepPlan dplan[3];
    std::vector<int> blk_first, wblk_first;
    double *xc_stage = nullptr;
    double *b_ext = nullptr;
    int n = 0;
// ... 31 lines not shown
    bool active = false, precond = false;
    const double *b = nullptr;
    double *x = nullptr;
    int count = 0;
    double r1 = 0.0;
};

struct F32Level {
    SdiaF32 A;
    float *csr_val = nullptr;
    float *diag = nullptr, *x = nullptr, *x2 = nullptr, *b = nullptr, *r = nullptr;
};

struct GraphState {
    hipGraph_t graph = nullptr;
    hipGraphExec_t exec = nullptr;
    double *x = nullptr;
    bool precond = false;
};

struct ProfileData {
    bool enabled = false;
    std::vector<hipEvent_t> ev;
    std::vector<int> run_launches;
    size_t used = 0;
    double launches = 0, seconds = 0;
};

class Engine {
public:
    Engine(int nrow, int ncol, const int *rowptr, const int *col, const double *val);
    ~Engine();

    int setup_host(const sparsh_params &p);
    int setup_host_shared(const sparsh_params &p);
    void set_share_setup(bool on) { share_setup_ = on; }
    bool built_locally() const { return built_locally_; }
    size_t shared_image_bytes() const { return image_bytes_; }
    int setup(const sparsh_params &p);
    bool ready() const { return ready_; }
    bool host_ready() const { return host_ready_; }
    int nlevels() const { return (int)lev_.size(); }
    const HostHierarchy &host() const { return H_; }
    const CoarseSolver &coarse() const { return coarse_; }
    CoarseSolver &coarse_mut() { return coarse_; }
    const sparsh_params &params() const { return prm_; }
    void set_smoother(int kind, int sweeps, int order);
    int smoother() const { return smoother_; }
    bool sor_on() const { return smoother_ == SPARSH_SMOOTH_SOR; }
    int sor_sweeps() const { return sm_sweeps_ > 0 ? sm_sweeps_ : kSorDefaultSweeps; }
    int sor_order() const { return sor_order_; }
    void set_sor_path(int mode) { sor_path_ = mode; }
    const ColorClasses &level_colors(int l);
    int sor_prepare();
    const SorLevel *sor_level(int l) const { return l >= 0 && l < (int)sor_.size() && sor_[l].rows ? &sor_[l] : nullptr; }
    bool sor_single(int l) const { return sor_path_ == 2 || (sor_path_ == 0 && sor_[l].single); }
    void sor_leg(int l, const double *b, double *x, int sweeps, bool reverse);
    bool op_sor(int l, const double *b, double *x, int sweeps, bool reverse, bool x_is_zero);
    bool build_sor_layouts();
    bool build_sor_level(int l);
    static constexpr int kSorDefaultSweeps = 6;
    static constexpr long kSorSingleNnz = 0;
    KernelConfig &kernel_cfg() { return cfg_; }
    const KernelConfig &kernel_cfg() const { return cfg_; }
    void config_changed() { drop_graph(); }
    const double *diag_stream(const DevLevel &L) const { return cfg_.const_diag && L.diag_is_const ? nullptr : L.diag; }
    bool zero_start(const DevLevel &L) const { return cfg_.zero_start && (!dist_ || L.replicated) && !L.deep && box2_applies(L.A, cfg_); }
    bool level_prolong_fused(int l) const
    {
        if (l < 1 || l + 1 >= (int)lev_.size() || !cfg_.fuse_prolong || prm_.sweeps < 1 || prm_.precond_fp32) return false;
        const DevLevel &F = lev_[l - 1];
        if (dist_ && !F.replicated) return false;
        return F.P_is_aggregation && !F.deep && (F.pair_aggregates || F.members) && F.R.nrow == lev_[l].n;
    }
    int level_paired(int l) const
    {
        if (!(l + 2 < (int)lev_.size() && prm_.sweeps > 0 && (!dist_ || lev_[l].replicated) && cfg_.pair_restrict)) return 0;
        if (lev_[l].pair_aggregates && resid_pair_applies(lev_[l].A, cfg_)) return 1;
        if (lev_[l].pair_axis != 0 && lev_[l].A.box_nx > 0 && csr_family(lev_[l].A, cfg_) == FAM_SDIA_TAB) return 1 + std::abs(lev_[l].pair_axis);
        return 0;
    }
    double bench_comm(int what, int level, int reps);
    hipStream_t stream() const { return st_; }
    const DevLevel &level(int l) const { return lev_[l]; }
    int n0() const { return A0_.nrow; }
    int local_n0() const { return lev_.empty() ? A0_.nrow : lev_[0].n; }
    void set_comm(std::unique_ptr<Comm> c) { comm_ = std::move(c); }
    void set_overlap(bool on) { overlap_ = on; }
    void set_deep_halo(bool on) { deep_halo_ = on; }
    bool deep_halo() const { return deep_halo_; }
    void set_comm_tuning(int mode) { comm_tune_ = mode; }
    struct CommLevelChoice {
        int rows = 0, halo_rows = 0;
        bool partitioned = false, deep = false;
        double cost_deep_us = 0.0, cost_per_sweep_us = 0.0, cost_replicated_us = 0.0;
    };
    struct CommMeasured {
        double exchange_us = 0.0, exchange_us_per_mb = 0.0, allreduce_us = 0.0, allgather_us = 0.0, allgather_us_per_mb = 0.0;
        double sweep_floor_us = 0.0, sweep_us_per_mb = 0.0;
        bool valid = false;
    };
    void plan_comm_schedule(const sparsh_params &p, int nranks, const CommMeasured &m)
    {
        meas_ = m;
        meas_.valid = true;
        sched_.clear();
        tuned_repl_level_ = -1;
        decide_comm_schedule(p, nranks);
    }
    int tuned_partitioned_levels() const { return tuned_repl_level_; }
    const std::vector<CommLevelChoice> &comm_schedule() const { return sched_; }
    const CommMeasured &comm_measured() const { return meas_; }
    long exchanges_issued() const { return n_exchanges_; }
    bool debug_prefix_spmv(int l, int rows, const double *x_ext, double *y);
    bool overlap() const { return overlap_; }
    Comm *comm() const { return comm_.get(); }
    bool distributed() const { return dist_; }
    bool precond_fp32_active() const { return f32_ready_; }
    const Partition &partition(int l) const { return parts_[l]; }
    void set_stopping(double tol, int max_iter, int check_every)
    {
        prm_.tol = tol;
        if (max_iter > 0) prm_.max_iter = max_iter;
        if (check_every > 0) prm_.check_every = check_every;
    }

    int solve_dev(int method, const double *b_dev, double *x_dev, int max_iters, double *hist, int hist_cap, int *iters,
                  double *seconds);
    int amg_solve_dev(const double *b_dev, double *x_dev, int iterations, double *hist, int hist_cap, int *ncycles);

    int pcg_init(const double *b_dev, double *x_dev, bool precond);
    int pcg_steps(int nsteps, int *done);
    int krylov_hist(double *hist, int hist_cap);
    double krylov_residual() const { return ks_.r1; }

    void op_spmv(int l, const double *x, double *y);
    void op_jacobi(int l, const double *b, double *x, double *tmp, int sweeps, bool x_is_zero);
    void op_residual(int l, const double *b, const double *x, double *r);
    double op_resnorm(int l, const double *b, const double *x);
    double op_spmv_dot(int l, const double *x, double *y);
    double op_jacobi_dot(int l, const double *b, const double *x, double *y);
    int set_box_plan(int l, int kernel, int q, int ty, int cz);
    bool op_restrict(int l, const double *r, double *bc, bool fuse_zero = false);
    void op_residual_restrict(int l, const double *b, const double *x, double *bc, double *xc);
    void op_jacobi_prolong(int l, const double *b, const double *x, double *xf);
    void op_prolong(int l, const double *xc, double *xf);
    void op_coarse(const double *b, double *x);
    bool op_precond_f32(const double *r, double *z);
    int op_precond(const double *r, double *z);
    static constexpr int kGmresDefaultRestart = 30;
    int set_gmres(int restart);
    int gmres_restart() const { return gm_restart_; }
    int set_gmres_basis(int precision);
    int gmres_basis() const { return gm_prec_; }
    size_t gmres_basis_bytes() const { return gm_bytes_; }
    int gmres_bench_prepare();
    void gmres_bench_step(bool fused);
    double op_dot(int n, const double *x, const double *y);

    void *dalloc(size_t bytes);
    void dfree(void *p);
    bool check(hipError_t e, const char *what);
    std::string error;
    int fault() const { return fault_; }
    bool note_hip(hipError_t e, const char *what);
    bool note_comm(bool ok, const char *what);

    ProfileData prof;
    void profile_begin();
    void profile_collect();
    double setup_seconds = 0.0;
    double place_best_us = 0.0, place_worst_us = 0.0, place_first_us = 0.0;
    int place_tried = 0;
    double place_seconds = 0.0;

private:
    void vcycle(const double *b0, bool x0_zero, double *dot_partial, int *dot_nblk, bool zero_done0 = false);
    void smooth(DevLevel &L, const double *b, int sweeps, bool x_zero, double *dot_partial, int *dot_nblk, bool zero_done = false,
                DevLevel *prolong_to = nullptr);
    bool halo(const DevPlan &p, double *vec);
    bool deep_exchange(DevLevel &L, int which, double *vec);
    int launch_prefix(DevLevel &L, int rows, CsrOp op, const CsrArgs &a);
    bool upload_deep_plan(const DeepPlan &h, DevDeepPlan &d);
    int apply_A(DevLevel &L, CsrOp op, CsrArgs a);
    void finalize(Fin code, const double *p0, const double *p1, int nblk, int slot, double *hist, int it, int nblk1 = -1);
    bool upload_plan(const HaloPlan &h, DevPlan &d);
    double read_scalar(int slot);
    double read_hist(int it);

    void vcycle_sor(const double *b0, bool x0_zero, double *dot_partial, int *dot_nblk);
    void adopt_sweeps();
    int pcg_smoother_check();
    int smoother_ = SPARSH_SMOOTH_JACOBI;
    int sm_sweeps_ = 0;
    int sor_order_ = SPARSH_SOR_FORWARD;
    int sor_path_ = 0;
    int base_sweeps_ = 0;
    std::vector<ColorClasses> colors_;
    std::vector<SorLevel> sor_;
    bool setup_f32();
    void vcycle_f32(const double *r64, double *z64, double *partial, int *nblk);
    void pcg_body(bool precond, int slot);
    bool capture_graph(bool precond);
    void drop_graph();
    int pcg(const double *b, double *x, int max_iters, double *hist, int hist_cap, int *iters, bool precond);
    int bicg(const double *b, double *x, int max_iters, double *hist, int hist_cap, int *iters, bool precond);
    int gmres(const double *b, double *x, int max_iters, double *hist, int hist_cap, int *iters, bool precond);
    int gmres_reserve();
    void gmres_release();
    void gmres_orthogonalise(int j, int slot, double *feed);
    double *gm_vec(int k) const { return gm_basis_ + (size_t)k * gm_stride_; }
    float *gm_vecf(int k) const { return gm_basisf_ + (size_t)k * gm_stride_; }
    int gm_restart_ = kGmresDefaultRestart;
    int gm_prec_ = SPARSH_BASIS_FP64;
    double *gm_basis_ = nullptr, *gm_part_ = nullptr, *gm_state_ = nullptr;
    float *gm_basisf_ = nullptr;
    double *gm_w_ = nullptr;
    GmresState gm_;
    long gm_stride_ = 0;
    size_t gm_bytes_ = 0;

    std::unique_ptr<Comm> comm_;
    std::vector<Partition> parts_;
    Partition gather_part_;
    int repl_level_ = 0;
// ... 50 lines not shown
```

sparsh_amg_amd/csrc/kernels.hip:

```cpp
#include <hip/hip_runtime.h>

#include "kernels.hpp"

#include <algorithm>
#include <vector>

namespace sparsh {

namespace {


__device__ __forceinline__ double wave_sum(double v)
{
#pragma unroll
    for (int off = 32; off > 0; off >>= 1) v += __shfl_down(v, off, 64);
    return v;
}

__device__ __forceinline__ double block_sum(double v, double *red)
{
    v = wave_sum(v);
    const int lane = threadIdx.x & 63, w = threadIdx.x >> 6;
    if (lane == 0) red[w] = v;
    __syncthreads();
// ... 1025 lines not shown
    double acc = 0.0;
#pragma unroll
    for (int s = 0; s < S; ++s) {
        if (!valid[s]) continue;
        const int r = row[s];
        double sum = 0.0;
        if (conform[s]) {
            const int li = lo + (r - r0);
            double xv[ND];
            if constexpr (ND == 7) {
                xv[0] = xm[s];
                xv[6] = xp[s];
            }
            xv[C0 - 2] = xt[li - lo];
            xv[C0 - 1] = xt[li - 1];
            xv[C0] = xc[s];
            xv[C0 + 1] = xt[li + 1];
            xv[C0 + 2] = xt[li + hi];
#pragma unroll
            for (int u = 0; u < ND; ++u) {
                const bool on = __builtin_amdgcn_inverse_ballot_w64(m[s][u]);
                const double t = tab.cval[u] * xv[u];
                sum = on ? sum + t : sum;
            }
            o[s].di = __builtin_amdgcn_inverse_ballot_w64(m[s][C0]) ? tab.cval[C0] : 0.0;
            if constexpr (op_needs_xi(OP)) o[s].xi = xc[s];
        } else {
            if constexpr (op_needs_xi(OP)) o[s].xi = xc[s];
            sum = sdia_offtable_row<false>(r >> 6, r, lane, x, sd_ptr, sd_off, sd_mask, sd_vidx, sd_cval, sd_val, sd_rec, o[s].di);
        }
        if (has_row[s]) acc += row_epilogue<OP>(a, r, sum, o[s]);
    }
    if constexpr (op_reduces(OP)) {
        acc = wave_sum(acc);
        if (lane == 0) red[w] = acc;
        __syncthreads();
        if (threadIdx.x == 0) {
            double t = 0.0;
#pragma unroll
            for (int q = 0; q < NW; ++q) t += red[q];
            a.partial[a.partial_off + tile] = t;
        }
    }
}

constexpr int kBoxBlock = 1024;

struct DivConst {
    double b, bs0, r0;
};
__device__ __forceinline__ DivConst make_div_const(double b)
{
    DivConst c;
    c.b = b;
    bool f;
    c.bs0 = __builtin_amdgcn_div_scale(1.0, b, false, &f);
    double r = __builtin_amdgcn_rcp(c.bs0);
    double e = __builtin_fma(-c.bs0, r, 1.0);
    r = __builtin_fma(r, e, r);
    e = __builtin_fma(-c.bs0, r, 1.0);
    r = __builtin_fma(r, e, r);
    c.r0 = r;
    return c;
}
__device__ __forceinline__ double div_const(double a, const DivConst &c)
{
    bool fd, fn;
    const double bs = __builtin_amdgcn_div_scale(a, c.b, false, &fd);
    const double as = __builtin_amdgcn_div_scale(a, c.b, true, &fn);
    if (__builtin_amdgcn_ballot_w64(bs != c.bs0) != 0ull) return a / c.b;
    const double q0 = as * c.r0;
    const double rem = __builtin_fma(-bs, q0, as);
    const double q = __builtin_amdgcn_div_fmas(rem, c.r0, q0, fn);
    return __builtin_amdgcn_div_fixup(q, c.b, a);
}

struct BoxArgs {
    int nx, ny, nz;
    int TY, CZ, ytiles;
    double c[7];
    double omega;
};

template <int Q, int TAG, bool ZERO>
__global__ __launch_bounds__(kBoxBlock) void sdia_box2_kernel(BoxArgs g, const double *__restrict__ x, const double *__restrict__ b,
                                                               double *__restrict__ y)
{
    extern __shared__ double box_lds[];
    const int nx = g.nx, ny = g.ny, nz = g.nz, P = nx * ny, TY = g.TY;
    const int R0 = (TY + 4) * nx;
    const int pitch = nx + 1;
    const int cells = (TY + 4) * pitch + 1;
    double *X0 = box_lds;
    double *X1 = box_lds + cells;
    int wg = blockIdx.x;
    {
        const int nwg = gridDim.x, per = nwg / 8, rem = nwg % 8;
        const int c = wg % 8, r = wg / 8;
        wg = c * per + min(c, rem) + r;
    }
    const int tile = wg % g.ytiles, zc = wg / g.ytiles;
    const int j0 = tile * TY;
    const int z0 = zc * g.CZ, z1 = min(z0 + g.CZ, nz);
    const long base = (long)(j0 - 2) * nx;
    const int tid = threadIdx.x;
    const double c0 = g.c[0], c1 = g.c[1], c2 = g.c[2], c3 = g.c[3], c4 = g.c[4], c5 = g.c[5], c6 = g.c[6], om = g.omega;
    const DivConst dc = make_div_const(c3);
    for (int i = tid; i < 2 * cells; i += kBoxBlock) box_lds[i] = 0.0;
    bool v0[Q], v1[Q], v2[Q];
    int sidx[Q];
    double xm[Q], xc[Q], xp[Q], bk[Q], bp[Q], x1m[Q], x1c[Q];
    double bq[Q];
#pragma unroll
    for (int q = 0; q < Q; ++q) {
        const int p = tid + kBoxBlock * q;
        const int lr = p / nx;
        const int jr = j0 - 2 + lr;
        sidx[q] = p + lr + 1;
        v0[q] = p < R0 && jr >= 0 && jr < ny;
        v1[q] = v0[q] && lr >= 1 && lr <= TY + 2;
        v2[q] = v0[q] && lr >= 2 && lr <= TY + 1;
        xm[q] = xc[q] = xp[q] = bk[q] = bp[q] = x1m[q] = x1c[q] = bq[q] = 0.0;
    }
    const int ks = z0 - 1;
#pragma unroll
    for (int q = 0; q < Q; ++q) {
        const int p = tid + kBoxBlock * q;
        if constexpr (ZERO) {
            if (v0[q]) {
                if (ks >= 1) xm[q] = div_const(om * b[(long)(ks - 1) * P + base + p], dc);
                if (ks >= 0) {
                    bk[q] = b[(long)ks * P + base + p];
                    xc[q] = div_const(om * bk[q], dc);
                }
                if (ks + 1 < nz) {
                    bq[q] = b[(long)(ks + 1) * P + base + p];
                    xp[q] = div_const(om * bq[q], dc);
                }
            }
        } else {
            if (v0[q]) {
                if (ks >= 1) xm[q] = x[(long)(ks - 1) * P + base + p];
                if (ks >= 0) xc[q] = x[(long)ks * P + base + p];
                if (ks + 1 < nz) xp[q] = x[(long)(ks + 1) * P + base + p];
            }
            if (v1[q] && ks >= 0) bk[q] = b[(long)ks * P + base + p];
        }
    }
    __syncthreads();
    for (int k = ks; k <= z1; ++k) {
        const bool plane = k >= 0 && k < nz;
        double xn[Q], bn[Q];
#pragma unroll
        for (int q = 0; q < Q; ++q) {
            const int p = tid + kBoxBlock * q;
            xn[q] = 0.0;
            bn[q] = 0.0;
            if (k + 1 <= z1) {
                if constexpr (ZERO) {
                    if (v0[q] && k + 2 < nz) xn[q] = b[(long)(k + 2) * P + base + p];
                } else {
                    if (v0[q] && k + 2 < nz) xn[q] = x[(long)(k + 2) * P + base + p];
                    if (v1[q] && k + 1 < nz) bn[q] = b[(long)(k + 1) * P + base + p];
                }
            }
        }
#pragma unroll
        for (int q = 0; q < Q; ++q)
            if (v0[q]) X0[sidx[q]] = xc[q];
        __syncthreads();
        double x1k[Q];
#pragma unroll
        for (int q = 0; q < Q; ++q) {
            x1k[q] = 0.0;
            if (plane && v1[q]) {
                const int s = sidx[q];
                double sum = 0.0;
                sum = sum + c0 * xm[q];
                sum = sum + c1 * X0[s - pitch];
                sum = sum + c2 * X0[s - 1];
                sum = sum + c3 * xc[q];
                sum = sum + c4 * X0[s + 1];
                sum = sum + c5 * X0[s + pitch];
                sum = sum + c6 * xp[q];
                const double h = 1.0 * bk[q] + (-1.0) * sum;
                x1k[q] = xc[q] + div_const(om * h, dc);
            }
        }
        const int k2 = k - 1;
        if (k2 >= z0 && k2 < z1) {
#pragma unroll
            for (int q = 0; q < Q; ++q) {
                const int p = tid + kBoxBlock * q;
                if (v2[q]) {
                    const int s = sidx[q];
                    double sum = 0.0;
                    sum = sum + c0 * x1m[q];
                    sum = sum + c1 * X1[s - pitch];
                    sum = sum + c2 * X1[s - 1];
                    sum = sum + c3 * x1c[q];
                    sum = sum + c4 * X1[s + 1];
                    sum = sum + c5 * X1[s + pitch];
                    sum = sum + c6 * x1k[q];
                    const double h = 1.0 * bp[q] + (-1.0) * sum;
                    y[(long)k2 * P + base + p] = x1c[q] + div_const(om * h, dc);
                }
            }
        }
        __syncthreads();
#pragma unroll
        for (int q = 0; q < Q; ++q) {
            if (v1[q]) X1[sidx[q]] = x1k[q];
            x1m[q] = x1c[q];
            x1c[q] = x1k[q];
            xm[q] = xc[q];
            xc[q] = xp[q];
            bp[q] = bk[q];
            if constexpr (ZERO) {
                bk[q] = bq[q];
                bq[q] = xn[q];
                xp[q] = 0.0;
                if (v0[q] && k + 1 <= z1 && k + 2 < nz) xp[q] = div_const(om * xn[q], dc);
            } else {
                xp[q] = xn[q];
                bk[q] = bn[q];
            }
        }
    }
}

enum BoxEpi : int { BOX_SPMV_DOT = 0, BOX_JACOBI_DOT = 1, BOX_RESID_PAIRX = 2, BOX_JACOBI_PROLONG = 3, BOX_JACOBI = 4 };

struct Box1Args {
    const double *x, *b;
    double *y;
    double *y2;
    const double *dc;
    double dconst;
    const int *members;
    int nfine;
    double *partial;
};

template <int Q, int EPI, int TAG>
__global__ __launch_bounds__(kBoxBlock) void sdia_box1_kernel(BoxArgs g, Box1Args a)
{
    extern __shared__ double box_lds[];
    __shared__ double red[kBoxBlock / 64];
    const int nx = g.nx, ny = g.ny, nz = g.nz, P = nx * ny, TY = g.TY;
    const int R0 = (TY + 2) * nx;
    const int pitch = nx + 1;
    const int cells = (TY + 2) * pitch + 1;
    double *X0 = box_lds;
    int wg = blockIdx.x;
    {
        const int nwg = gridDim.x, per = nwg / 8, rem = nwg % 8;
        const int c = wg % 8, r = wg / 8;
        wg = c * per + min(c, rem) + r;
    }
    const int tile = wg % g.ytiles, zc = wg / g.ytiles;
    const int j0 = tile * TY;
    const int z0 = zc * g.CZ, z1 = min(z0 + g.CZ, nz);
    const long base = (long)(j0 - 1) * nx;
    const int tid = threadIdx.x;
    const double c0 = g.c[0], c1 = g.c[1], c2 = g.c[2], c3 = g.c[3], c4 = g.c[4], c5 = g.c[5], c6 = g.c[6], om = g.omega;
    constexpr bool kNeedsB = EPI != BOX_SPMV_DOT;
    constexpr bool kDivides = EPI == BOX_JACOBI_DOT || EPI == BOX_JACOBI_PROLONG || EPI == BOX_JACOBI;
    DivConst dc3 = {1.0, 1.0, 1.0};
    if constexpr (kDivides) dc3 = make_div_const(c3);
    for (int i = tid; i < cells; i += kBoxBlock) X0[i] = 0.0;
    bool v0[Q], v1[Q];
    int sidx[Q];
    double xm[Q], xc[Q], xp[Q], bk[Q];
#pragma unroll
    for (int q = 0; q < Q; ++q) {
        const int p = tid + kBoxBlock * q;
        const int lr = p / nx;
        const int jr = j0 - 1 + lr;
        sidx[q] = p + lr + 1;
        v0[q] = p < R0 && jr >= 0 && jr < ny;
        v1[q] = v0[q] && lr >= 1 && lr <= TY;
        xm[q] = xc[q] = xp[q] = bk[q] = 0.0;
        if (v0[q]) {
            if (z0 >= 1) xm[q] = a.x[(long)(z0 - 1) * P + base + p];
            xc[q] = a.x[(long)z0 * P + base + p];
            if (z0 + 1 < nz) xp[q] = a.x[(long)(z0 + 1) * P + base + p];
        }
        if constexpr (kNeedsB) {
            if (v1[q]) bk[q] = a.b[(long)z0 * P + base + p];
        }
    }
    __syncthreads();
    double acc = 0.0;
    for (int k = z0; k < z1; ++k) {
        double xn[Q], bn[Q];
#pragma unroll
        for (int q = 0; q < Q; ++q) {
            const int p = tid + kBoxBlock * q;
            xn[q] = 0.0;
            bn[q] = 0.0;
            if (k + 1 < z1) {
                if (v0[q] && k + 2 < nz) xn[q] = a.x[(long)(k + 2) * P + base + p];
                if constexpr (kNeedsB) {
                    if (v1[q]) bn[q] = a.b[(long)(k + 1) * P + base + p];
                }
            }
        }
#pragma unroll
        for (int q = 0; q < Q; ++q)
            if (v0[q]) X0[sidx[q]] = xc[q];
        __syncthreads();
#pragma unroll
        for (int q = 0; q < Q; ++q) {
            const int p = tid + kBoxBlock * q;
            const int s = sidx[q];
            const long row = (long)k * P + base + p;
            double sum = 0.0;
            if (v1[q]) {
                sum = sum + c0 * xm[q];
                sum = sum + c1 * X0[s - pitch];
                sum = sum + c2 * X0[s - 1];
                sum = sum + c3 * xc[q];
                sum = sum + c4 * X0[s + 1];
                sum = sum + c5 * X0[s + pitch];
                sum = sum + c6 * xp[q];
            }
            if constexpr (EPI == BOX_SPMV_DOT) {
                if (v1[q]) {
                    a.y[row] = sum;
                    acc += xc[q] * sum;
                }
            } else if constexpr (EPI == BOX_JACOBI_DOT || EPI == BOX_JACOBI) {
                if (v1[q]) {
                    const double h = 1.0 * bk[q] + (-1.0) * sum;
                    const double xnew = xc[q] + div_const(om * h, dc3);
                    a.y[row] = xnew;
                    if constexpr (EPI == BOX_JACOBI_DOT) acc += xnew * bk[q];
                }
            } else if constexpr (EPI == BOX_JACOBI_PROLONG) {
                if (v1[q]) {
                    const double h = 1.0 * bk[q] + (-1.0) * sum;
                    const double xnew = xc[q] + div_const(om * h, dc3);
                    if (a.members) {
                        const i2v m = *reinterpret_cast<const i2v *>(a.members + 2 * row);
                        a.y2[m.x] = 1.0 * xnew + a.y2[m.x];
                        if (m.y >= 0) a.y2[m.y] = 1.0 * xnew + a.y2[m.y];
                    } else {
                        const long f = 2 * row;
                        if (f + 1 < a.nfine) {
                            d2v *pp = reinterpret_cast<d2v *>(a.y2 + f);
                            d2v v = *pp;
                            v.x = 1.0 * xnew + v.x;
                            v.y = 1.0 * xnew + v.y;
                            *pp = v;
                        } else {
                            a.y2[f] = 1.0 * xnew + a.y2[f];
                        }
                    }
                }
            } else {
                const double ri = v1[q] ? 1.0 * bk[q] + (-1.0) * sum : 0.0;
                const double rn = lane_from_above(ri, 0.0);
                if (v1[q] && !(tid & 1)) {
                    const long J = row >> 1;
                    double bc = 0.0 + ri;
                    bc = bc + rn;
                    a.y[J] = bc;
                    if (a.y2) a.y2[J] = om * bc / (a.dc ? a.dc[J] : a.dconst);
                }
            }
        }
        __syncthreads();
#pragma unroll
        for (int q = 0; q < Q; ++q) {
            xm[q] = xc[q];
            xc[q] = xp[q];
            xp[q] = xn[q];
            bk[q] = bn[q];
        }
    }
    if constexpr (EPI == BOX_SPMV_DOT || EPI == BOX_JACOBI_DOT) {
        acc = wave_sum(acc);
        const int lane = tid & 63, w = tid >> 6;
        if (lane == 0) red[w] = acc;
        __syncthreads();
        if (tid == 0) {
            double t = 0.0;
#pragma unroll
            for (int q = 0; q < kBoxBlock / 64; ++q) t += red[q];
            a.partial[blockIdx.x] = t;
        }
    }
}

__device__ __forceinline__ double box_residual(const BoxArgs &g, const double *__restrict__ x, const double *__restrict__ b, int f, int i, int j,
                                               int k)
{
    const int nx = g.nx, P = g.nx * g.ny;
    const double xm2 = k > 0 ? x[f - P] : 0.0;
    const double xm1 = j > 0 ? x[f - nx] : 0.0;
    const double xm0 = i > 0 ? x[f - 1] : 0.0;
    const double xc = x[f];
    const double xp0 = i < nx - 1 ? x[f + 1] : 0.0;
    const double xp1 = j < g.ny - 1 ? x[f + nx] : 0.0;
    const double xp2 = k < g.nz - 1 ? x[f + P] : 0.0;
    const double bi = b[f];
    double sum = 0.0;
    sum = sum + g.c[0] * xm2;
    sum = sum + g.c[1] * xm1;
    sum = sum + g.c[2] * xm0;
    sum = sum + g.c[3] * xc;
    sum = sum + g.c[4] * xp0;
    sum = sum + g.c[5] * xp1;
    sum = sum + g.c[6] * xp2;
    return 1.0 * bi + (-1.0) * sum;
}

template <int AXIS>
__global__ __launch_bounds__(kBlock) void box_resid_pair_kernel(BoxArgs g, int nc, int rev, const double *__restrict__ x, const double *__restrict__ b,
                                                                const double *__restrict__ dc, double dconst, double *__restrict__ bc,
                                                                double *__restrict__ xc)
{
    const int J = blockIdx.x * kBlock + threadIdx.x;
    if (J >= nc) return;
    const int nx = g.nx, ny = g.ny;
    const int cny = AXIS == 1 ? ny / 2 : ny;
    const int i = J % nx, t = J / nx;
    const int cj = t % cny, ck = t / cny;
    const int j = AXIS == 1 ? 2 * cj : cj, k = AXIS == 2 ? 2 * ck : ck;
    const int f1 = i + nx * (j + ny * k);
    const int f2 = f1 + (AXIS == 1 ? nx : nx * ny);
    const int Jout = rev ? nc - 1 - J : J;
    const double dj = !xc ? 1.0 : (dc ? dc[Jout] : dconst);
    const double r1 = box_residual(g, x, b, f1, i, j, k);
    const double r2 = box_residual(g, x, b, f2, i, j + (AXIS == 1 ? 1 : 0), k + (AXIS == 2 ? 1 : 0));
    double s = 0.0 + r1;
    s = s + r2;
    bc[Jout] = s;
    if (xc) xc[Jout] = g.omega * s / dj;
}

template <int L>
__device__ __forceinline__ float sdia32_chunk(const int *__restrict__ off, const unsigned long long *__restrict__ mask,
                                              const float *__restrict__ vp, const float *__restrict__ x, int d0, int row, int lane,
                                              float &dv, float sum)
{
    float v[L], xv[L];
    bool on[L];
    int oo[L];
#pragma unroll
    for (int u = 0; u < L; ++u) {
        const int o = __builtin_amdgcn_readfirstlane(off[d0 + u]);
        oo[u] = o;
        const unsigned long long m = mask[d0 + u];
        on[u] = (m >> lane) & 1ull;
        v[u] = vp[(size_t)(d0 + u) * 64];
        xv[u] = x[on[u] ? row + o : row];
    }
#pragma unroll
    for (int u = 0; u < L; ++u) {
        const float t = v[u] * xv[u];
        sum = on[u] ? sum + t : sum;
        if (oo[u] == 0) dv = on[u] ? v[u] : dv;
    }
    return sum;
}

template <int OP>
__global__ __launch_bounds__(kBlock) void sdia_f32_kernel(int nrow, int nslice, int ngroups, int remap, const int *__restrict__ sd_ptr,
                                                           const int *__restrict__ sd_off, const unsigned long long *__restrict__ sd_mask,
                                                           const float *__restrict__ sd_val, const float *__restrict__ x,
                                                           const float *__restrict__ b, float *__restrict__ y, float omega)
// ... 193 lines not shown
        return A.nblk;
    }
#define SPARSH_LAUNCH_BLOCK(NT_, VEC_) \
    hipLaunchKernelGGL((csr_block_kernel<OP, NT_, VEC_, TAG>), dim3(grid), dim3(kBlock), 0, st, A.rowblk, A.nblk, remap, A.rowptr, A.col, A.val, a)
    if (nt && c.vec) SPARSH_LAUNCH_BLOCK(true, 1);
    else if (nt) SPARSH_LAUNCH_BLOCK(true, 0);
    else if (c.vec) SPARSH_LAUNCH_BLOCK(false, 1);
    else SPARSH_LAUNCH_BLOCK(false, 0);
#undef SPARSH_LAUNCH_BLOCK
    return A.nblk;
}

}

namespace {
size_t box2_lds_bytes(int nx, int TY) { return (size_t)2 * ((size_t)(TY + 4) * (nx + 1) + 1) * sizeof(double); }
size_t box1_lds_bytes(int nx, int TY) { return ((size_t)(TY + 2) * (nx + 1) + 1) * sizeof(double); }
}

bool box2_plan(DevCsr &A)
{
    A.box_q = A.box_ty = A.box_cz = 0;
    const int nx = A.box_nx, ny = A.box_ny, nz = A.box_nz;
    if (nx < 2 || ny < 1 || nz < 1) return false;
    long best = -1;
    for (int Q = 2; Q <= 4; ++Q) {
        int TY = std::min(ny, Q * kBoxBlock / nx - 4);
        while (TY >= 1 && box2_lds_bytes(nx, TY) > 65536) --TY;
        if (TY < 1) continue;
        const int ytiles = (ny + TY - 1) / TY;
        for (int zch = 1; zch <= nz; ++zch) {
            const int CZ = (nz + zch - 1) / zch;
            const int chunks = (nz + CZ - 1) / CZ;
            const long wgs = (long)ytiles * chunks;
            long cost;
            if (Q == 2 && wgs > 256) cost = ((wgs + 511) / 512) * (CZ + 2) * Q * 16;
            else cost = ((wgs + 255) / 256) * (CZ + 2) * Q * 10;
            if (best < 0 || cost < best) {
                best = cost;
                A.box_q = Q;
                A.box_ty = TY;
                A.box_cz = CZ;
            }
        }
    }
    return A.box_q > 0;
}

bool box1_plan(DevCsr &A, bool shared_cu)
{
    A.box1_q = A.box1_ty = A.box1_cz = 0;
    const int nx = A.box_nx, ny = A.box_ny, nz = A.box_nz;
    if (nx < 2 || ny < 1 || nz < 1) return false;
    long best = -1;
    for (int Q = 2; Q <= 4; ++Q) {
        int TY = std::min(ny, Q * kBoxBlock / nx - 2);
        while (TY >= 1 && box1_lds_bytes(nx, TY) > 65536) --TY;
        if (TY < 1) continue;
        const int ytiles = (ny + TY - 1) / TY;
        for (int zch = 1; zch <= nz; ++zch) {
            const int CZ = (nz + zch - 1) / zch;
            const int chunks = (nz + CZ - 1) / CZ;
            const long wgs = (long)ytiles * chunks;
            long cost;
            if (shared_cu && Q <= 3 && wgs > 256) cost = ((wgs + 511) / 512) * (CZ + 1) * Q * 16;
            else cost = ((wgs + 255) / 256) * (CZ + 1) * Q * 10;
            if (best < 0 || cost < best) {
                best = cost;
                A.box1_q = Q;
                A.box1_ty = TY;
                A.box1_cz = CZ;
            }
        }
    }
    return A.box1_q > 0;
}

int box1_workgroups(const DevCsr &A)
{
    if (A.box1_q <= 0 || A.box1_ty <= 0 || A.box1_cz <= 0) return 0;
    return ((A.box_ny + A.box1_ty - 1) / A.box1_ty) * ((A.box_nz + A.box1_cz - 1) / A.box1_cz);
}

const char *box_plan_refusal(const DevCsr &A, int kernel, int Q, int TY, int CZ)
{
    const int nx = A.box_nx, ny = A.box_ny, nz = A.box_nz;
    if (nx <= 0) return "the level is not a box grid";
    if (kernel != 1 && kernel != 2) return "kernel must be 2 (double sweep) or 1 (plane-marching kernel)";
    if (Q < 2 || Q > 4) return "points per thread must be 2, 3 or 4";
    if (TY < 1 || TY > ny) return "lines per tile must lie in 1 .. ny";
    if (CZ < 1 || CZ > nz) return "planes per chunk must lie in 1 .. nz";
    const int halo = kernel == 2 ? 4 : 2;
    if ((long)(TY + halo) * nx > (long)Q * kBoxBlock) return "the tile's region has more points than the workgroup's threads hold";
    if ((kernel == 2 ? box2_lds_bytes(nx, TY) : box1_lds_bytes(nx, TY)) > 65536) return "the tile's region does not fit the 64 KiB of LDS";
    return nullptr;
}

bool box1_applies(const DevCsr &A, const KernelConfig &c)
{
    return c.box1 != 0 && A.box1_on && A.box1_q > 0 && csr_family(A, c) == FAM_SDIA_TAB;
}

int launch_box1(const DevCsr &A, int epi, const CsrArgs &a, bool finest, hipStream_t st)
{
    BoxArgs g;
    g.nx = A.box_nx;
    g.ny = A.box_ny;
    g.nz = A.box_nz;
    g.TY = A.box1_ty;
    g.CZ = A.box1_cz;
    g.ytiles = (g.ny + g.TY - 1) / g.TY;
    for (int u = 0; u < 7; ++u) g.c[u] = A.sd_tab.cval[u];
    g.omega = a.omega;
    Box1Args b;
    b.x = a.x;
    b.b = a.b;
    b.y = a.y;
    b.y2 = a.y2;
    b.dc = a.d;
    b.dconst = a.dconst;
    b.members = a.members;
    b.nfine = a.nfine;
    b.partial = a.partial ? a.partial + a.partial_off : nullptr;
    const int chunks = (g.nz + g.CZ - 1) / g.CZ;
    const int nwg = g.ytiles * chunks;
    const dim3 grid(nwg), block(kBoxBlock);
    const size_t lds = box1_lds_bytes(g.nx, g.TY);
#define SPARSH_LAUNCH_BOX1(Q_, E_)                                                                  \
    do {                                                                                            \
        if (finest) hipLaunchKernelGGL((sdia_box1_kernel<Q_, E_, 1>), grid, block, lds, st, g, b);  \
        else hipLaunchKernelGGL((sdia_box1_kernel<Q_, E_, 0>), grid, block, lds, st, g, b);         \
    } while (0)
#define SPARSH_LAUNCH_BOX1_Q(E_)                      \
    do {                                              \
        if (A.box1_q == 4) SPARSH_LAUNCH_BOX1(4, E_); \
        else if (A.box1_q == 3) SPARSH_LAUNCH_BOX1(3, E_); \
        else SPARSH_LAUNCH_BOX1(2, E_);               \
    } while (0)
    switch (epi) {
    case BOX_SPMV_DOT: SPARSH_LAUNCH_BOX1_Q(BOX_SPMV_DOT); break;
    case BOX_JACOBI_DOT: SPARSH_LAUNCH_BOX1_Q(BOX_JACOBI_DOT); break;
    case BOX_RESID_PAIRX: SPARSH_LAUNCH_BOX1_Q(BOX_RESID_PAIRX); break;
    case BOX_JACOBI: SPARSH_LAUNCH_BOX1_Q(BOX_JACOBI); break;
    default: SPARSH_LAUNCH_BOX1_Q(BOX_JACOBI_PROLONG); break;
    }
#undef SPARSH_LAUNCH_BOX1_Q
#undef SPARSH_LAUNCH_BOX1
    return nwg;
}

bool box2_applies(const DevCsr &A, const KernelConfig &c)
{
    return c.box2 != 0 && A.box_on && A.box_q > 0 && csr_family(A, c) == FAM_SDIA_TAB;
}

void launch_box2(const DevCsr &A, const double *x, const double *b, double *y, double omega, bool finest, hipStream_t st, bool from_zero)
{
    BoxArgs g;
    g.nx = A.box_nx;
    g.ny = A.box_ny;
    g.nz = A.box_nz;
    g.TY = A.box_ty;
    g.CZ = A.box_cz;
    g.ytiles = (g.ny + g.TY - 1) / g.TY;
    for (int u = 0; u < 7; ++u) g.c[u] = A.sd_tab.cval[u];
    g.omega = omega;
    const int chunks = (g.nz + g.CZ - 1) / g.CZ;
    const dim3 grid(g.ytiles * chunks), block(kBoxBlock);
    const size_t lds = box2_lds_bytes(g.nx, g.TY);
#define SPARSH_LAUNCH_BOX(Q_)                                                                                       \
    do {                                                                                                            \
        if (from_zero) {                                                                                            \
            if (finest) hipLaunchKernelGGL((sdia_box2_kernel<Q_, 1, true>), grid, block, lds, st, g, x, b, y);      \
            else hipLaunchKernelGGL((sdia_box2_kernel<Q_, 0, true>), grid, block, lds, st, g, x, b, y);             \
        } else {                                                                                                    \
            if (finest) hipLaunchKernelGGL((sdia_box2_kernel<Q_, 1, false>), grid, block, lds, st, g, x, b, y);     \
            else hipLaunchKernelGGL((sdia_box2_kernel<Q_, 0, false>), grid, block, lds, st, g, x, b, y);            \
        }                                                                                                           \
    } while (0)
    if (A.box_q == 4) SPARSH_LAUNCH_BOX(4);
    else if (A.box_q == 3) SPARSH_LAUNCH_BOX(3);
    else SPARSH_LAUNCH_BOX(2);
#undef SPARSH_LAUNCH_BOX
}

void launch_box_resid_pair(const DevCsr &A, int axis, const double *x, const double *b, const double *dc, double dconst, double omega,
                           double *bc, double *xc, hipStream_t st)
{
    BoxArgs g;
    g.nx = A.box_nx;
    g.ny = A.box_ny;
    g.nz = A.box_nz;
    g.TY = g.CZ = g.ytiles = 0;
    for (int u = 0; u < 7; ++u) g.c[u] = A.sd_tab.cval[u];
    g.omega = omega;
    const int nc = A.nrow / 2;
    if (nc <= 0) return;
    const dim3 grid((nc + kBlock - 1) / kBlock), block(kBlock);
    const int rev = axis < 0 ? 1 : 0;
    if (axis == 1 || axis == -1)
        hipLaunchKernelGGL(box_resid_pair_kernel<1>, grid, block, 0, st, g, nc, rev, x, b, dc, dconst, bc, xc);
    else
        hipLaunchKernelGGL(box_resid_pair_kernel<2>, grid, block, 0, st, g, nc, rev, x, b, dc, dconst, bc, xc);
}

bool resid_pair_applies(const DevCsr &A, const KernelConfig &c)
{
    return c.pair_restrict && csr_family(A, c) == FAM_SDIA_TAB && sdia_tile_rows(A, c) == 0 && A.nslice > 0;
}

void launch_resid_pair(const DevCsr &A, const CsrArgs &a, bool finest, hipStream_t st, const KernelConfig &c)
{
    bool nt;
    int remap;
    csr_placement(A, c, &nt, &remap);
    const int ngroups = (A.nslice + 3) / 4;
    const int grid = remap_grid(ngroups, remap);
    if (finest)
        hipLaunchKernelGGL((sdia_tab_kernel<OP_RESID_PAIR, false, 1>), dim3(grid), dim3(kBlock), 0, st, A.nrow, A.ncol, A.nslice, ngroups, remap, A.sd_tab, nullptr, A.sd_tmask, A.sd_tconf, A.sd_ptr, A.sd_off, A.sd_mask, A.sd_vidx, A.sd_cval, A.sd_val, A.sd_rec, a);
    else
        hipLaunchKernelGGL((sdia_tab_kernel<OP_RESID_PAIR, false, 0>), dim3(grid), dim3(kBlock), 0, st, A.nrow, A.ncol, A.nslice, ngroups, remap, A.sd_tab, nullptr, A.sd_tmask, A.sd_tconf, A.sd_ptr, A.sd_off, A.sd_mask, A.sd_vidx, A.sd_cval, A.sd_val, A.sd_rec, a);
}

CsrFamily csr_family(const DevCsr &A, const KernelConfig &c)
{
    if (c.kind == 3 && A.has_sdia() && c.table && A.sd_tmask) return FAM_SDIA_TAB;
    const bool small_prefers_ell = A.sell_val && A.nrow < 65536;
    if (c.kind == 3 && A.has_sdia() && !small_prefers_ell) return FAM_SDIA;
    if (c.kind >= 2 && A.sell_val) return FAM_SELL;
    if (c.kind == 1 && A.waveblk) return FAM_CSR_WAVE;
    const size_t csr_bytes = (size_t)A.nnz * 12 + (size_t)A.nrow * 36;
    const bool streams = csr_bytes > (240u << 20);
    if ((c.vec == 4 || (c.vec == 3 && streams)) && A.col16) return FAM_CSR_ROWLANE16;
    if (c.vec == 2 || c.vec == 4 || (c.vec == 3 && streams)) return FAM_CSR_ROWLANE;
    return FAM_CSR_BLOCK;
}

bool csr_alternates(const DevCsr &A, const KernelConfig &c)
{
    if (c.alt_dir == 0) return false;
    if (c.alt_dir >= 2) return true;
    size_t bytes = (size_t)A.nrow * 24;
    switch (csr_family(A, c)) {
    case FAM_SDIA_TAB: break;
    case FAM_SDIA: bytes += (size_t)A.sd_vblocks * 64 * 8; break;
    case FAM_SELL: bytes += (size_t)A.sell_entries * 12; break;
    case FAM_CSR_ROWLANE16: bytes += (size_t)A.nnz * 10; break;
    default: bytes += (size_t)A.nnz * 12; break;
    }
    return bytes > ((size_t)640 << 20);
}

int sdia_tile_rows(const DevCsr &A, const KernelConfig &c)
{
    if (!c.tile || !A.sd_tmask || (A.sd_tab.near != 73 && A.sd_tab.near != 52)) return 0;
    const int C0 = A.sd_tab.nd / 2;
    const int lo = -A.sd_tab.off[C0 - 2], hi = A.sd_tab.off[C0 + 2];
    if (lo < 2 || hi < 2) return 0;
    if (A.sd_tab.nd == 7 && (-A.sd_tab.off[0] <= lo || A.sd_tab.off[6] <= hi)) return 0;
    if (A.nrow < 65536) return 0;
    const int reach = lo + hi;
    const int T = reach <= 512 ? 1024 : (reach <= 1024 ? 2048 : (reach <= 2048 ? 4096 : 0));
    return T;
}

// ... 846 lines not shown
```

sparsh_amg_amd/csrc/kernels.hpp:

```cpp
#pragma once

#include <hip/hip_runtime_api.h>

#include <vector>

namespace sparsh {

struct SdTable {
    int nd = 0;
    int near = 0;
    int off[8] = {0, 0, 0, 0, 0, 0, 0, 0};
    double cval[8] = {0, 0, 0, 0, 0, 0, 0, 0};
};

struct DevCsr {
    int nrow = 0, ncol = 0, nnz = 0;
    int *rowptr = nullptr;
    int *col = nullptr;
    double *val = nullptr;
    int *rowblk = nullptr;
    int nblk = 0;
    unsigned short *col16 = nullptr;
    int *cbase = nullptr;
    int nblk16 = 0;
    int *waveblk = nullptr;
    int nwblk = 0;
    int nslice = 0;
    int *slice_ptr = nullptr;
    int *sell_col = nullptr;
    double *sell_val = nullptr;
    long sell_entries = 0;
    int *sd_ptr = nullptr;
    int *sd_off = nullptr;
    unsigned long long *sd_mask = nullptr;
    double *sd_val = nullptr;
    long sd_slots = 0;
    int *sd_vidx = nullptr;
    double *sd_cval = nullptr;
    long sd_vblocks = 0;
    int *sd_rec = nullptr;
    SdTable sd_tab;
    unsigned long long *sd_tmask = nullptr;
    int *sd_tconf = nullptr;
    bool has_sdia() const { return sd_ptr != nullptr; }
    int box_nx = 0, box_ny = 0, box_nz = 0;
    int box_q = 0, box_ty = 0, box_cz = 0;
    bool box_on = false;
    int box1_q = 0, box1_ty = 0, box1_cz = 0;
    bool box1_on = false;
    int *int_list = nullptr, *bnd_list = nullptr;
    int nint = 0, nbnd = 0;
};

struct KernelConfig {
    int kind = 3;
    int vec = 3;
    bool auto_policy = true;
    bool nt = true;
    int remap = 1;
    bool table = true;
    bool tile = false;
    bool const_slots = true;
    bool place_search = true;
    bool cg_nt = true;
    bool fuse_cg_zero = true;
    int alt_dir = 1;
    bool defer_x = true;
    bool zero_start = true;
    int box1 = 1;
    int box2 = 1;
    bool const_diag = true;
    bool fuse_prolong = true;
    bool pair_restrict = true;
    int idx16 = 1;
};

enum CsrFamily : int { FAM_CSR_BLOCK = 0, FAM_CSR_WAVE = 1, FAM_SELL = 2, FAM_SDIA = 3, FAM_SDIA_TAB = 4, FAM_CSR_ROWLANE = 5, FAM_CSR_ROWLANE16 = 6 };

constexpr int kBlock = 256;
constexpr int kStreamNnz = 2048;
constexpr int kWaveNnz = 512;
constexpr int kSdRecInts = 48;
constexpr int kSdConstBit = 1 << 30;
constexpr int kSdPlainBit = 1 << 29;
constexpr int kSdPtrMask = (1 << 29) - 1;
constexpr int kCsrPad = 4;

enum CsrOp : int {
    OP_SPMV = 0,
    OP_RESID = 1,
    OP_JACOBI = 2,
    OP_ADD = 3,
    OP_SPMV_DOT = 4,
    OP_RESNORM = 5,
    OP_JACOBI_DOT = 6,
    OP_JACOBI_PROLONG = 8,
    OP_RESID_PAIR = 7
};

struct CsrArgs {
    const double *x = nullptr;
    const double *b = nullptr;
    const double *d = nullptr;
    double *y = nullptr;
    double *y2 = nullptr;
    double dconst = 0.0;
    const int *members = nullptr;
    int nfine = 0;
    double omega = 0.0;
    double *partial = nullptr;
    const int *slice_list = nullptr;
    int nlist = 0;
    int partial_off = 0;
    int reverse = 0;
};

int build_rowblocks(int nrow, const int *rowptr, int *out);
int build_waveblocks(int nrow, const int *rowptr, int *out);
std::vector<int> rowblock_records(int nrow, const int *rowptr, int *nblk);
int build_col16(const int *rowptr, const int *col, const int *rec, int nblk, unsigned short *col16, int *cbase);

int launch_csr(const DevCsr &A, CsrOp op, const CsrArgs &a, bool finest, hipStream_t st, const KernelConfig &cfg);
CsrFamily csr_family(const DevCsr &A, const KernelConfig &cfg);
bool box2_plan(DevCsr &A);
bool box2_applies(const DevCsr &A, const KernelConfig &cfg);
void launch_box2(const DevCsr &A, const double *x, const double *b, double *y, double omega, bool finest, hipStream_t st, bool from_zero = false);
void launch_box_resid_pair(const DevCsr &A, int axis, const double *x, const double *b, const double *dc, double dconst, double omega,
                           double *bc, double *xc, hipStream_t st);
bool box1_plan(DevCsr &A, bool shared_cu = false);
bool box1_applies(const DevCsr &A, const KernelConfig &cfg);
int box1_workgroups(const DevCsr &A);
const char *box_plan_refusal(const DevCsr &A, int kernel, int Q, int TY, int CZ);
int launch_box1(const DevCsr &A, int epi, const CsrArgs &a, bool finest, hipStream_t st);
bool resid_pair_applies(const DevCsr &A, const KernelConfig &cfg);
void launch_resid_pair(const DevCsr &A, const CsrArgs &a, bool finest, hipStream_t st, const KernelConfig &cfg);
bool csr_alternates(const DevCsr &A, const KernelConfig &cfg);
const char *csr_family_name(CsrFamily f);
int sdia_tile_rows(const DevCsr &A, const KernelConfig &cfg);
void csr_placement(const DevCsr &A, const KernelConfig &cfg, bool *nt, int *remap);

void launch_jacobi_zero(int n, const double *b, const double *d, double dconst, double omega, double *x, hipStream_t st);
void launch_prolong_agg(int n, const int *agg, const double *xc, double *xf, hipStream_t st);
void launch_restrict_agg(int nc, const int *rowptr, const int *col, const double *r, double *bc, hipStream_t st);
void launch_restrict_agg_zero(int nc, const int *rowptr, const int *col, const double *r, double *bc, const double *dc, double dconst,
                              double omega, double *xc, hipStream_t st);
void launch_gemv(int n, const double *M, const double *b, double *x, hipStream_t st);

struct SorArgs {
    const int *rows = nullptr;
    const int *rowptr = nullptr;
    const int *col = nullptr;
    const double *val = nullptr;
    const double *diag = nullptr;
    const double *b = nullptr;
    double *x = nullptr;
    double omega = 0.0;
};
void launch_sor_colour(const int *rec, int nblk, bool nt, const SorArgs &a, hipStream_t st);
void launch_sor_level(const int *cstart, int ncolors, int sweeps, bool reverse, const SorArgs &a, hipStream_t st);

void launch_fill(int n, double v, double *x, hipStream_t st);
void launch_copy(int n, const double *x, double *y, hipStream_t st);
void launch_copy_int(int n, const int *x, int *y, hipStream_t st);
void launch_spin(double microseconds, hipStream_t st);
void launch_axpby(int n, double a, const double *x, double b, double *y, hipStream_t st);
void launch_dot(int n, const double *x, const double *y, double *partial, int *nblk, hipStream_t st);

struct SdiaF32 {
    int nrow = 0, nslice = 0;
    const int *sd_ptr = nullptr;
    const int *sd_off = nullptr;
    const unsigned long long *sd_mask = nullptr;
    float *val = nullptr;
    long slots = 0;
};
void launch_sdia_f32(const SdiaF32 &A, CsrOp op, const float *x, const float *b, float *y, float omega, hipStream_t st);
void launch_csr_f32(const DevCsr &A, const float *val32, CsrOp op, const float *diag, const float *x, const float *b, float *y, float omega,
                    hipStream_t st);
void launch_jacobi_zero_f32(int n, const float *b, const float *d, float omega, float *x, hipStream_t st);
void launch_restrict_f32(int nc, const int *rowptr, const int *col, const double *val, const float *r, float *bc, hipStream_t st);
void launch_prolong_agg_f32(int n, const int *agg, const float *xc, float *xf, hipStream_t st);
void launch_prolong_csr_f32(int n, const int *rowptr, const int *col, const double *val, const float *xc, float *xf, hipStream_t st);
void launch_gemv_f32(int n, const float *M, const float *b, float *x, hipStream_t st);
void launch_cvt_d2f(long n, const double *in, float *out, hipStream_t st);
void launch_cvt_f2d_dot(int n, const float *z32, const double *r64, double *z64, double *partial, int *nblk, hipStream_t st);

enum Slot : int {
    S_RZ = 0, S_PAP, S_ALPHA, S_NALPHA, S_BETA, S_RR, S_RES, S_ZR,
    S_ALPHA1, S_APR0, S_ASS, S_ASAS, S_OMEGA1, S_RR0, S_TMP, S_SUM0, S_SUM1, S_COUNT
};

enum Fin : int {
    FIN_STORE = 0,
    FIN_SQRT = 1,
    FIN_PCG_ALPHA = 2,
    FIN_PCG_BETA = 3,
    FIN_CG_BETA = 4,
    FIN_CG_ALPHA = 5,
    FIN_BICG_ALPHA = 6,
    FIN_BICG_OMEGA = 7,
    FIN_BICG_BETA = 8,
    FIN_PCG_BETA_RES = 9
};
void launch_finalize(Fin code, const double *partial0, const double *partial1, int nblk, double *scal, int slot_a,
                     double *hist, int it, hipStream_t st, int mode = 0, int *iter_ctr = nullptr, int hist_cap = 1 << 30,
                     int nblk1 = -1);
void launch_pack(int n, const int *idx, const double *vec, double *sendbuf, hipStream_t st);
void launch_unpack(int n, const int *pos, const double *buf, double *vec, hipStream_t st);

void launch_cg_update(int n, const double *scal, const double *p, const double *Ap, double *x, double *r, double *partial,
                      int *nblk, hipStream_t st);
void launch_cg_update_zero(int n, const double *scal, const double *p, const double *Ap, double *x, double *r, double *partial,
                           int *nblk, const double *d, double dconst, double omega, double *z0, hipStream_t st, bool nt = false);
void launch_p_update(int n, const double *scal, const double *z, double *p, hipStream_t st);
void launch_xp_update(int n, const double *scal, const double *z, double *p, double *x, hipStream_t st);
// ... 34 lines not shown
```

Baseline: 693.1.

## Autotune box kernel block size and tile plans on coarse levels

Templates the box double-sweep and plane-marching kernels on workgroup size (256/512/1024) and adds a candidate-plan generator. Setup timing then searches these plans on non-finest levels, and the minimum level size for tuning drops from 400k to 60k rows. Smaller coarse grids can pick plans that launch more workgroups, aiming to improve occupancy and parallelism there. The cost is longer setup and more template instantiations, plus a new benchmark op for the marching kernel.

```diff
diff --git a/include/sparsh_amg.h b/include/sparsh_amg.h
--- a/include/sparsh_amg.h
+++ b/include/sparsh_amg.h
@@ -82,6 +82,9 @@
 int sparsh_set_deferred_x(sparsh_handle h, int enable);
 int sparsh_level_marching_ops(sparsh_handle h, int level, int *on, int *plan, double *table_us, double *marching_us);
 int sparsh_set_box_plan(sparsh_handle h, int level, int kernel, int q, int ty, int cz);
+int sparsh_set_box_plan_ex(sparsh_handle h, int level, int kernel, int threads, int q, int ty, int cz);
+int sparsh_level_box_threads(sparsh_handle h, int level, int *double_threads, int *marching_threads);
+int sparsh_debug_box_plan_candidates(int kernel, int nx, int ny, int nz, int part_cap, int cap, int *plans);
 int sparsh_level_double_sweep(sparsh_handle h, int level, int *on, int *dims, int *plan, double *single_us, double *double_us);
 int sparsh_level_constant_diagonal(sparsh_handle h, int level, int *is_const, double *value);
 int sparsh_level_prolong_fused(sparsh_handle h, int level, int *fused);
diff --git a/sparsh_amg_amd/__init__.py b/sparsh_amg_amd/__init__.py
--- a/sparsh_amg_amd/__init__.py
+++ b/sparsh_amg_amd/__init__.py
@@ -100,6 +100,9 @@
         "sparsh_level_prolong_fused": (C.c_int, [H, C.c_int, C.POINTER(C.c_int)]),
         "sparsh_op_jacobi_prolong": (C.c_int, [H, C.c_int, c_dbl_p, c_dbl_p, c_dbl_p]),
         "sparsh_set_box_plan": (C.c_int, [H, C.c_int, C.c_int, C.c_int, C.c_int, C.c_int]),
+        "sparsh_set_box_plan_ex": (C.c_int, [H, C.c_int, C.c_int, C.c_int, C.c_int, C.c_int, C.c_int]),
+        "sparsh_level_box_threads": (C.c_int, [H, C.c_int, c_int_p, c_int_p]),
+        "sparsh_debug_box_plan_candidates": (C.c_int, [C.c_int, C.c_int, C.c_int, C.c_int, C.c_int, C.c_int, c_int_p]),
         "sparsh_op_spmv_dot": (C.c_int, [H, C.c_int, c_dbl_p, c_dbl_p, c_dbl_p]),
         "sparsh_op_jacobi_dot": (C.c_int, [H, C.c_int, c_dbl_p, c_dbl_p, c_dbl_p, c_dbl_p]),
         "sparsh_level_paired": (C.c_int, [H, C.c_int, C.POINTER(C.c_int)]),
@@ -259,6 +262,16 @@
     return a.value, b.value
 
 
+def box_plan_candidates(kernel, nx, ny, nz, part_cap=0):
+    k = {"double": 2, "marching": 1}.get(kernel, kernel)
+    cap = 64
+    buf = (C.c_int * (4 * cap))()
+    n = lib.sparsh_debug_box_plan_candidates(int(k), int(nx), int(ny), int(nz), int(part_cap), cap, buf)
+    if n < 0:
+        raise ValueError("kernel must be 2 (double sweep) or 1 (plane-marching kernel)")
+    return [tuple(buf[4 * i:4 * i + 4]) for i in range(min(n, cap))]
+
+
 def device_count() -> int:
     return lib.sparsh_device_count()
 
@@ -363,14 +376,19 @@
         return {"on": bool(on.value), "points_per_thread": plan[0], "lines_per_tile": plan[1], "planes_per_chunk": plan[2],
                 "table_kernel_us": round(t1.value, 2), "marching_kernel_us": round(t2.value, 2)}
 
-    def set_box_plan(self, level, kernel, q=0, ty=0, cz=0, shared_cu=False):
+    def set_box_plan(self, level, kernel, q=0, ty=0, cz=0, shared_cu=False, threads=1024):
         k = {"double": 2, "marching": 1}.get(kernel, kernel)
         if shared_cu:
             if k != 1:
                 raise ValueError("shared_cu is a plan of the marching kernel")
             k = 3
-        _check(lib.sparsh_set_box_plan(self._h, int(level), int(k), int(q), int(ty), int(cz)))
-        return self
+        _check(lib.sparsh_set_box_plan_ex(self._h, int(level), int(k), int(threads), int(q), int(ty), int(cz)))
+        return self
+
+    def level_box_threads(self, level):
+        a, b = C.c_int(0), C.c_int(0)
+        _check(lib.sparsh_level_box_threads(self._h, int(level), C.byref(a), C.byref(b)))
+        return a.value, b.value
 
     def set_constant_diagonal(self, enable=True):
         _check(lib.sparsh_set_constant_diagonal(self._h, 1 if enable else 0))
@@ -752,7 +770,7 @@
     def bench_op(self, op, level=0, reps=20):
         ops = {"spmv": 0, "jacobi": 1, "residual": 2, "restrict": 3, "prolong": 4, "coarse": 5, "dot": 6, "axpby": 7, "copy_int": 8,
                "jacobi_pingpong": 9, "jacobi_pingpong_resident": 10, "jacobi_double": 11, "sor": 12,
-               "gmres_orth": 13, "gmres_orth_unfused": 14, "gmres_orth_fp32_basis": 15}
+               "gmres_orth": 13, "gmres_orth_unfused": 14, "gmres_orth_fp32_basis": 15, "jacobi_dot_marching": 16}
         sec = C.c_double()
         _check(lib.sparsh_bench_op(self._h, ops[op] if isinstance(op, str) else op, level, reps, C.byref(sec)))
         return sec.value
diff --git a/sparsh_amg_amd/csrc/capi.cpp b/sparsh_amg_amd/csrc/capi.cpp
--- a/sparsh_amg_amd/csrc/capi.cpp
+++ b/sparsh_amg_amd/csrc/capi.cpp
@@ -476,12 +476,40 @@
     return SPARSH_OK;
 }
 
+int sparsh_set_box_plan_ex(sparsh_handle h, int level, int kernel, int threads, int q, int ty, int cz)
+{
+    REQUIRE_READY(h);
+    REQUIRE_LEVEL(h, level);
+    const int rc = h->eng->set_box_plan(level, kernel, threads, q, ty, cz);
+    return rc == SPARSH_OK ? SPARSH_OK : fail(rc, h->eng->error);
+}
+
 int sparsh_set_box_plan(sparsh_handle h, int level, int kernel, int q, int ty, int cz)
 {
-    REQUIRE_READY(h);
-    REQUIRE_LEVEL(h, level);
-    const int rc = h->eng->set_box_plan(level, kernel, q, ty, cz);
-    return rc == SPARSH_OK ? SPARSH_OK : fail(rc, h->eng->error);
+    return sparsh_set_box_plan_ex(h, level, kernel, 1024, q, ty, cz);
+}
+
+int sparsh_level_box_threads(sparsh_handle h, int level, int *double_threads, int *marching_threads)
+{
+    REQUIRE_READY(h);
+    REQUIRE_LEVEL(h, level);
+    const DevLevel &L = h->eng->level(level);
+    if (double_threads) *double_threads = L.A.box_q > 0 ? L.A.box_bs : 0;
+    if (marching_threads) *marching_threads = L.A.box1_q > 0 ? L.A.box1_bs : 0;
+    return SPARSH_OK;
+}
+
+int sparsh_debug_box_plan_candidates(int kernel, int nx, int ny, int nz, int part_cap, int cap, int *plans)
+{
+    if (kernel != 1 && kernel != 2) return -1;
+    const std::vector<BoxPlan> c = box_plan_candidates(kernel, nx, ny, nz, part_cap);
+    for (size_t i = 0; i < c.size() && (int)i < cap && plans; ++i) {
+        plans[4 * i] = c[i].threads;
+        plans[4 * i + 1] = c[i].q;
+        plans[4 * i + 2] = c[i].ty;
+        plans[4 * i + 3] = c[i].cz;
+    }
+    return (int)c.size();
 }
 
 int sparsh_set_constant_diagonal(sparsh_handle h, int enable)
@@ -1392,13 +1420,25 @@
             ++flip2;
             launch_box2(L.A, xa, L.r, xb, E.params().omega, L.fine, st);
         } break;
+        case 16: {
+            static thread_local int flip3 = 0;
+            CsrArgs a;
+            a.x = (flip3 & 1) ? L.x2 : L.x;
+            a.y = (flip3 & 1) ? L.x : L.x2;
+            ++flip3;
+            a.b = L.r;
+            a.d = L.diag;
+            a.omega = E.params().omega;
+            a.partial = E.partials();
+            launch_box1(L.A, 1, a, L.fine, st);
+        } break;
         case 13: E.gmres_bench_step(true); break;
         case 14: E.gmres_bench_step(false); break;
         case 15: E.gmres_bench_step(true); break;
         default: break;
         }
     };
-    if (op < 0 || op > 15) return fail(SPARSH_EINVAL, "unknown op");
+    if (op < 0 || op > 16) return fail(SPARSH_EINVAL, "unknown op");
     if (op == 13 || op == 14 || op == 15) {
         if (level != 0 || E.distributed()) return fail(SPARSH_EINVAL, "the GMRES orthogonalisation step runs on level 0 of a single-GPU handle");
         if ((op == 15) != (E.gmres_basis() == SPARSH_BASIS_FP32))
@@ -1407,6 +1447,8 @@
     }
     if (op == 12 && (E.distributed() || !E.build_sor_level(level))) return fail(SPARSH_ESTATE, "no SOR layout on this handle");
     if (op == 11 && (E.distributed() || !box2_applies(L.A, E.kernel_cfg()))) return fail(SPARSH_ESTATE, "the level does not run double sweeps (sparsh_level_double_sweep)");
+    if (op == 16 && (E.distributed() || !box1_applies(L.A, E.kernel_cfg()))) return fail(SPARSH_ESTATE, "the level does not run the plane-marching kernel (sparsh_level_marching_ops)");
+    if (op == 10 || op == 11 || op == 16) launch_fill(L.n, 1.0, L.r, st);
     for (int i = 0; i < 3; ++i) run();
     hipEvent_t e0, e1;
     (void)hipEventCreate(&e0);
@@ -1419,6 +1461,11 @@
     (void)hipEventElapsedTime(&ms, e0, e1);
     (void)hipEventDestroy(e0);
     (void)hipEventDestroy(e1);
+    if (op == 10 || op == 11 || op == 16) {
+        (void)hipMemsetAsync(L.x, 0, n * 8, st);
+        (void)hipMemsetAsync(L.x2, 0, n * 8, st);
+        (void)hipMemsetAsync(L.r, 0, n * 8, st);
+    }
     *avg_seconds = ms * 1e-3 / reps;
     return SPARSH_OK;
 }
diff --git a/sparsh_amg_amd/csrc/engine.cpp b/sparsh_amg_amd/csrc/engine.cpp
--- a/sparsh_amg_amd/csrc/engine.cpp
+++ b/sparsh_amg_amd/csrc/engine.cpp
@@ -591,6 +591,7 @@
 
 void Engine::tune_box_kernels()
 {
+    auto same_plan = [](const BoxPlan &a, const BoxPlan &b) { return a.threads == b.threads && a.q == b.q && a.ty == b.ty && a.cz == b.cz; };
     for (size_t l = 0; l + 1 < lev_.size(); ++l) {
         DevLevel &L = lev_[l];
         L.A.box_on = L.A.box1_on = false;
@@ -600,7 +601,7 @@
         if (cfg_.box1 >= 2) L.A.box1_on = L.A.box1_q > 0;
         const bool time2 = cfg_.box2 == 1, time1 = cfg_.box1 == 1 && L.A.box1_q > 0;
         if (!(time1 || time2)) continue;
-        if (L.n < 400000) continue;
+        if (L.n < 60000) continue;
         hipEvent_t e0 = nullptr, e1 = nullptr;
         if (hipEventCreate(&e0) != hipSuccess || hipEventCreate(&e1) != hipSuccess) continue;
         CsrArgs a;
@@ -631,6 +632,36 @@
         if (time2) {
             L.box_single_us = timed(false);
             L.box_double_us = timed(true);
+            const BoxPlan planned = {L.A.box_bs, L.A.box_q, L.A.box_ty, L.A.box_cz};
+            BoxPlan best = planned;
+            double t_best = 1e30;
+            std::vector<BoxPlan> others;
+            if (!L.fine) others = box_plan_candidates(2, L.A.box_nx, L.A.box_ny, L.A.box_nz, 0);
+            for (const BoxPlan &c : others) {
+                if (same_plan(c, planned)) continue;
+                L.A.box_bs = c.threads;
+                L.A.box_q = c.q;
+                L.A.box_ty = c.ty;
+                L.A.box_cz = c.cz;
+                const double t = std::min(timed(true), timed(true));
+                if (t < t_best) {
+                    t_best = t;
+                    best = c;
+                }
+            }
+            if (t_best < 1e30) {
+                L.A.box_bs = planned.threads;
+                L.A.box_q = planned.q;
+                L.A.box_ty = planned.ty;
+                L.A.box_cz = planned.cz;
+                L.box_double_us = std::min(L.box_double_us, timed(true));
+            }
+            if (!(t_best < 0.97 * L.box_double_us)) best = planned;
+            else L.box_double_us = t_best;
+            L.A.box_bs = best.threads;
+            L.A.box_q = best.q;
+            L.A.box_ty = best.ty;
+            L.A.box_cz = best.cz;
             L.A.box_on = L.box_double_us < 0.97 * L.box_single_us;
         }
         if (time1) {
@@ -669,6 +700,38 @@
                     L.A.box1_ty = ty0;
                     L.A.box1_cz = cz0;
                 }
+            }
+            {
+                const BoxPlan current = {L.A.box1_bs, L.A.box1_q, L.A.box1_ty, L.A.box1_cz};
+                auto set1 = [&](const BoxPlan &c) {
+                    L.A.box1_bs = c.threads;
+                    L.A.box1_q = c.q;
+                    L.A.box1_ty = c.ty;
+                    L.A.box1_cz = c.cz;
+                };
+                BoxPlan best = current;
+                double t_best = 1e30;
+                DevCsr T = L.A;
+                const bool has_planner = box1_plan(T);
+                const BoxPlan planner = {1024, T.box1_q, T.box1_ty, T.box1_cz};
+                std::vector<BoxPlan> others;
+                if (!L.fine) others = box_plan_candidates(1, L.A.box_nx, L.A.box_ny, L.A.box_nz, part_cap_);
+                for (const BoxPlan &c : others) {
+                    if ((has_planner && same_plan(c, planner)) || same_plan(c, current)) continue;
+                    set1(c);
+                    const double t = std::min(timed1(true), timed1(true));
+                    if (t < t_best) {
+                        t_best = t;
+                        best = c;
+                    }
+                }
+                if (t_best < 1e30) {
+                    set1(current);
+                    L.box1_us = std::min(L.box1_us, timed1(true));
+                }
+                if (t_best < 0.97 * L.box1_us) L.box1_us = t_best;
+                else best = current;
+                set1(best);
             }
             L.A.box1_on = L.box1_us < 0.97 * L.box1_table_us;
         }
@@ -1315,6 +1378,7 @@
     place_best_us = place_worst_us = place_first_us = 0.0;
     phase("coarsest-level factorisation + workspace");
     tune_box_kernels();
+    phase("box kernel plans");
     if (G == 1 && cfg_.place_search) tune_placement();
     phase("placement search");
     f32_ready_ = false;
@@ -1616,7 +1680,7 @@
     return read_scalar(S_TMP);
 }
 
-int Engine::set_box_plan(int l, int kernel, int q, int ty, int cz)
+int Engine::set_box_plan(int l, int kernel, int threads, int q, int ty, int cz)
 {
     auto refuse = [&](const std::string &why) {
         error = why;
@@ -1629,13 +1693,15 @@
     if (kernel == 3 && !planner) return refuse("kernel 3 takes the planner's shared-CU plan: q, ty and cz must be 0");
     DevCsr T = A;
     if (planner) {
+        threads = 1024;
         if (!(kernel == 2 ? box2_plan(T) : box1_plan(T, kernel == 3))) return refuse("the planner has no plan for this grid");
         q = kernel == 2 ? T.box_q : T.box1_q;
         ty = kernel == 2 ? T.box_ty : T.box1_ty;
         cz = kernel == 2 ? T.box_cz : T.box1_cz;
     }
-    if (const char *why = box_plan_refusal(A, kernel == 2 ? 2 : 1, q, ty, cz)) return refuse(why);
+    if (const char *why = box_plan_refusal(A, kernel == 2 ? 2 : 1, threads, q, ty, cz)) return refuse(why);
     if (kernel == 2) {
+        A.box_bs = threads;
         A.box_q = q;
         A.box_ty = ty;
         A.box_cz = cz;
@@ -1645,6 +1711,7 @@
         T.box1_cz = cz;
         if (box1_workgroups(T) > part_cap_)
             return refuse("the plan launches " + std::to_string(box1_workgroups(T)) + " workgroups; the partial buffers hold " + std::to_string(part_cap_));
+        A.box1_bs = threads;
         A.box1_q = q;
         A.box1_ty = ty;
         A.box1_cz = cz;
diff --git a/sparsh_amg_amd/csrc/engine.hpp b/sparsh_amg_amd/csrc/engine.hpp
--- a/sparsh_amg_amd/csrc/engine.hpp
+++ b/sparsh_amg_amd/csrc/engine.hpp
@@ -137,6 +137,7 @@
     }
     double bench_comm(int what, int level, int reps);
     hipStream_t stream() const { return st_; }
+    double *partials() const { return part0_; }
     const DevLevel &level(int l) const { return lev_[l]; }
     int n0() const { return A0_.nrow; }
     int local_n0() const { return lev_.empty() ? A0_.nrow : lev_[0].n; }
@@ -195,7 +196,7 @@
     double op_resnorm(int l, const double *b, const double *x);
     double op_spmv_dot(int l, const double *x, double *y);
     double op_jacobi_dot(int l, const double *b, const double *x, double *y);
-    int set_box_plan(int l, int kernel, int q, int ty, int cz);
+    int set_box_plan(int l, int kernel, int threads, int q, int ty, int cz);
     bool op_restrict(int l, const double *r, double *bc, bool fuse_zero = false);
     void op_residual_restrict(int l, const double *b, const double *x, double *bc, double *xc);
     void op_jacobi_prolong(int l, const double *b, const double *x, double *xf);
diff --git a/sparsh_amg_amd/csrc/kernels.hip b/sparsh_amg_amd/csrc/kernels.hip
--- a/sparsh_amg_amd/csrc/kernels.hip
+++ b/sparsh_amg_amd/csrc/kernels.hip
@@ -1131,9 +1131,9 @@
     double omega;
 };
 
-template <int Q, int TAG, bool ZERO>
-__global__ __launch_bounds__(kBoxBlock) void sdia_box2_kernel(BoxArgs g, const double *__restrict__ x, const double *__restrict__ b,
-                                                               double *__restrict__ y)
+template <int BS, int Q, int TAG, bool ZERO>
+__global__ __launch_bounds__(BS) void sdia_box2_kernel(BoxArgs g, const double *__restrict__ x, const double *__restrict__ b,
+                                                        double *__restrict__ y)
 {
     extern __shared__ double box_lds[];
     const int nx = g.nx, ny = g.ny, nz = g.nz, P = nx * ny, TY = g.TY;
@@ -1155,14 +1155,14 @@
     const int tid = threadIdx.x;
     const double c0 = g.c[0], c1 = g.c[1], c2 = g.c[2], c3 = g.c[3], c4 = g.c[4], c5 = g.c[5], c6 = g.c[6], om = g.omega;
     const DivConst dc = make_div_const(c3);
-    for (int i = tid; i < 2 * cells; i += kBoxBlock) box_lds[i] = 0.0;
+    for (int i = tid; i < 2 * cells; i += BS) box_lds[i] = 0.0;
     bool v0[Q], v1[Q], v2[Q];
     int sidx[Q];
     double xm[Q], xc[Q], xp[Q], bk[Q], bp[Q], x1m[Q], x1c[Q];
     double bq[Q];
 #pragma unroll
     for (int q = 0; q < Q; ++q) {
-        const int p = tid + kBoxBlock * q;
+        const int p = tid + BS * q;
         const int lr = p / nx;
         const int jr = j0 - 2 + lr;
         sidx[q] = p + lr + 1;
@@ -1174,7 +1174,7 @@
     const int ks = z0 - 1;
 #pragma unroll
     for (int q = 0; q < Q; ++q) {
-        const int p = tid + kBoxBlock * q;
+        const int p = tid + BS * q;
         if constexpr (ZERO) {
             if (v0[q]) {
                 if (ks >= 1) xm[q] = div_const(om * b[(long)(ks - 1) * P + base + p], dc);
@@ -1202,7 +1202,7 @@
         double xn[Q], bn[Q];
 #pragma unroll
         for (int q = 0; q < Q; ++q) {
-            const int p = tid + kBoxBlock * q;
+            const int p = tid + BS * q;
             xn[q] = 0.0;
             bn[q] = 0.0;
             if (k + 1 <= z1) {
@@ -1240,7 +1240,7 @@
         if (k2 >= z0 && k2 < z1) {
 #pragma unroll
             for (int q = 0; q < Q; ++q) {
-                const int p = tid + kBoxBlock * q;
+                const int p = tid + BS * q;
                 if (v2[q]) {
                     const int s = sidx[q];
                     double sum = 0.0;
@@ -1291,11 +1291,11 @@
     double *partial;
 };
 
-template <int Q, int EPI, int TAG>
-__global__ __launch_bounds__(kBoxBlock) void sdia_box1_kernel(BoxArgs g, Box1Args a)
+template <int BS, int Q, int EPI, int TAG>
+__global__ __launch_bounds__(BS) void sdia_box1_kernel(BoxArgs g, Box1Args a)
 {
     extern __shared__ double box_lds[];
-    __shared__ double red[kBoxBlock / 64];
+    __shared__ double red[BS / 64];
     const int nx = g.nx, ny = g.ny, nz = g.nz, P = nx * ny, TY = g.TY;
     const int R0 = (TY + 2) * nx;
     const int pitch = nx + 1;
@@ -1317,13 +1317,13 @@
     constexpr bool kDivides = EPI == BOX_JACOBI_DOT || EPI == BOX_JACOBI_PROLONG || EPI == BOX_JACOBI;
     DivConst dc3 = {1.0, 1.0, 1.0};
     if constexpr (kDivides) dc3 = make_div_const(c3);
-    for (int i = tid; i < cells; i += kBoxBlock) X0[i] = 0.0;
+    for (int i = tid; i < cells; i += BS) X0[i] = 0.0;
     bool v0[Q], v1[Q];
     int sidx[Q];
     double xm[Q], xc[Q], xp[Q], bk[Q];
 #pragma unroll
     for (int q = 0; q < Q; ++q) {
-        const int p = tid + kBoxBlock * q;
+        const int p = tid + BS * q;
         const int lr = p / nx;
         const int jr = j0 - 1 + lr;
         sidx[q] = p + lr + 1;
@@ -1345,7 +1345,7 @@
         double xn[Q], bn[Q];
 #pragma unroll
         for (int q = 0; q < Q; ++q) {
-            const int p = tid + kBoxBlock * q;
+            const int p = tid + BS * q;
             xn[q] = 0.0;
             bn[q] = 0.0;
             if (k + 1 < z1) {
@@ -1361,7 +1361,7 @@
         __syncthreads();
 #pragma unroll
         for (int q = 0; q < Q; ++q) {
-            const int p = tid + kBoxBlock * q;
+            const int p = tid + BS * q;
             const int s = sidx[q];
             const long row = (long)k * P + base + p;
             double sum = 0.0;
@@ -1436,7 +1436,7 @@
         if (tid == 0) {
             double t = 0.0;
 #pragma unroll
-            for (int q = 0; q < kBoxBlock / 64; ++q) t += red[q];
+            for (int q = 0; q < BS / 64; ++q) t += red[q];
             a.partial[blockIdx.x] = t;
         }
     }
@@ -1796,18 +1796,100 @@
     return ((A.box_ny + A.box1_ty - 1) / A.box1_ty) * ((A.box_nz + A.box1_cz - 1) / A.box1_cz);
 }
 
-const char *box_plan_refusal(const DevCsr &A, int kernel, int Q, int TY, int CZ)
+const char *box_plan_refusal(const DevCsr &A, int kernel, int threads, int Q, int TY, int CZ)
 {
     const int nx = A.box_nx, ny = A.box_ny, nz = A.box_nz;
     if (nx <= 0) return "the level is not a box grid";
     if (kernel != 1 && kernel != 2) return "kernel must be 2 (double sweep) or 1 (plane-marching kernel)";
+    if (threads != 256 && threads != 512 && threads != 1024) return "threads per workgroup must be 256, 512 or 1024";
     if (Q < 2 || Q > 4) return "points per thread must be 2, 3 or 4";
     if (TY < 1 || TY > ny) return "lines per tile must lie in 1 .. ny";
     if (CZ < 1 || CZ > nz) return "planes per chunk must lie in 1 .. nz";
     const int halo = kernel == 2 ? 4 : 2;
-    if ((long)(TY + halo) * nx > (long)Q * kBoxBlock) return "the tile's region has more points than the workgroup's threads hold";
+    if ((long)(TY + halo) * nx > (long)Q * threads) return "the tile's region has more points than the workgroup's threads hold";
     if ((kernel == 2 ? box2_lds_bytes(nx, TY) : box1_lds_bytes(nx, TY)) > 65536) return "the tile's region does not fit the 64 KiB of LDS";
     return nullptr;
+}
+
+static long box_candidate_cost(int kernel, int nx, int ny, int nz, const BoxPlan &p)
+{
+    const long lds = (long)(kernel == 2 ? box2_lds_bytes(nx, p.ty) : box1_lds_bytes(nx, p.ty));
+    const int waves_simd = p.q == 2 ? 8 : (kernel == 2 ? (p.q == 3 ? 5 : 4) : (p.q == 3 ? 7 : 5));
+    long r = std::min<long>(2048 / p.threads, (long)waves_simd * 256 / p.threads);
+    r = std::max<long>(1, std::min<long>(r, 163840 / lds));
+    const long wgs = (long)((ny + p.ty - 1) / p.ty) * ((nz + p.cz - 1) / p.cz);
+    const long rounds = (wgs + 256 * r - 1) / (256 * r);
+    const long resident = std::min<long>(r, (wgs + 255) / 256);
+    return rounds * (p.cz + (kernel == 2 ? 2 : 1)) * (1536 + resident * p.q * p.threads);
+}
+
+std::vector<BoxPlan> box_plan_candidates(int kernel, int nx, int ny, int nz, int part_cap)
+{
+    std::vector<BoxPlan> out;
+    if ((kernel != 1 && kernel != 2) || nx < 2 || ny < 1 || nz < 1) return out;
+    DevCsr T;
+    T.box_nx = nx;
+    T.box_ny = ny;
+    T.box_nz = nz;
+    const int halo = kernel == 2 ? 4 : 2;
+    auto add = [&](int threads, int q, int ty, int cz) {
+        if (box_plan_refusal(T, kernel, threads, q, ty, cz)) return;
+        if (kernel == 1 && part_cap > 0 && (long)((ny + ty - 1) / ty) * ((nz + cz - 1) / cz) > part_cap) return;
+        for (const BoxPlan &o : out)
+            if (o.threads == threads && o.q == q && o.ty == ty && o.cz == cz) return;
+        out.push_back({threads, q, ty, cz});
+    };
+    if (kernel == 2 ? box2_plan(T) : box1_plan(T)) {
+        if (kernel == 2) add(kBoxBlock, T.box_q, T.box_ty, T.box_cz);
+        else add(kBoxBlock, T.box1_q, T.box1_ty, T.box1_cz);
+    }
+    if (kernel == 1 && box1_plan(T, true)) add(kBoxBlock, T.box1_q, T.box1_ty, T.box1_cz);
+    const size_t first = out.size();
+    for (int threads : {1024, 512, 256}) {
+        for (int Q = 2; Q <= 4; ++Q) {
+            int top = std::min(ny, Q * threads / nx - halo);
+            while (top >= 1 && (kernel == 2 ? box2_lds_bytes(nx, top) : box1_lds_bytes(nx, top)) > 65536) --top;
+            if (top < 1) continue;
+            for (int TY : {top, std::max(1, top / 2)}) {
+                const int ytiles = (ny + TY - 1) / TY;
+                for (int target : {256, 512, 1024}) {
+                    const int chunks = std::max(1, std::min(nz, (target + ytiles / 2) / ytiles));
+                    add(threads, Q, TY, (nz + chunks - 1) / chunks);
+                }
+                add(threads, Q, TY, nz);
+            }
+        }
+    }
+    if ((int)out.size() > kBoxCandidates) {
+        const size_t n = out.size();
+        std::vector<long> cost(n, 0);
+        std::vector<char> keep(n, 0);
+        for (size_t i = 0; i < n; ++i) cost[i] = i < first ? 0 : box_candidate_cost(kernel, nx, ny, nz, out[i]);
+        std::vector<size_t> order;
+        for (size_t i = first; i < n; ++i) order.push_back(i);
+        std::stable_sort(order.begin(), order.end(), [&](size_t x, size_t y) { return cost[x] < cost[y]; });
+        size_t nkeep = first;
+        for (size_t i = 0; i < first; ++i) keep[i] = 1;
+        for (int threads : {1024, 512, 256})
+            for (size_t i : order)
+                if (out[i].threads == threads) {
+                    keep[i] = 1;
+                    ++nkeep;
+                    break;
+                }
+        for (size_t i : order) {
+            if ((int)nkeep >= kBoxCandidates) break;
+            if (!keep[i]) {
+                keep[i] = 1;
+                ++nkeep;
+            }
+        }
+        std::vector<BoxPlan> kept;
+        for (size_t i = 0; i < n; ++i)
+            if (keep[i]) kept.push_back(out[i]);
+        out.swap(kept);
+    }
+    return out;
 }
 
 bool box1_applies(const DevCsr &A, const KernelConfig &c)
@@ -1838,18 +1920,24 @@
     b.partial = a.partial ? a.partial + a.partial_off : nullptr;
     const int chunks = (g.nz + g.CZ - 1) / g.CZ;
     const int nwg = g.ytiles * chunks;
-    const dim3 grid(nwg), block(kBoxBlock);
+    const dim3 grid(nwg), block(A.box1_bs);
     const size_t lds = box1_lds_bytes(g.nx, g.TY);
-#define SPARSH_LAUNCH_BOX1(Q_, E_)                                                                  \
-    do {                                                                                            \
-        if (finest) hipLaunchKernelGGL((sdia_box1_kernel<Q_, E_, 1>), grid, block, lds, st, g, b);  \
-        else hipLaunchKernelGGL((sdia_box1_kernel<Q_, E_, 0>), grid, block, lds, st, g, b);         \
+#define SPARSH_LAUNCH_BOX1(BS_, Q_, E_)                                                                  \
+    do {                                                                                                 \
+        if (finest) hipLaunchKernelGGL((sdia_box1_kernel<BS_, Q_, E_, 1>), grid, block, lds, st, g, b);  \
+        else hipLaunchKernelGGL((sdia_box1_kernel<BS_, Q_, E_, 0>), grid, block, lds, st, g, b);         \
     } while (0)
-#define SPARSH_LAUNCH_BOX1_Q(E_)                      \
-    do {                                              \
-        if (A.box1_q == 4) SPARSH_LAUNCH_BOX1(4, E_); \
-        else if (A.box1_q == 3) SPARSH_LAUNCH_BOX1(3, E_); \
-        else SPARSH_LAUNCH_BOX1(2, E_);               \
+#define SPARSH_LAUNCH_BOX1_BS(Q_, E_)                                \
+    do {                                                             \
+        if (A.box1_bs == 256) SPARSH_LAUNCH_BOX1(256, Q_, E_);       \
+        else if (A.box1_bs == 512) SPARSH_LAUNCH_BOX1(512, Q_, E_);  \
+        else SPARSH_LAUNCH_BOX1(1024, Q_, E_);                       \
+    } while (0)
+#define SPARSH_LAUNCH_BOX1_Q(E_)                              \
+    do {                                                      \
+        if (A.box1_q == 4) SPARSH_LAUNCH_BOX1_BS(4, E_);      \
+        else if (A.box1_q == 3) SPARSH_LAUNCH_BOX1_BS(3, E_); \
+        else SPARSH_LAUNCH_BOX1_BS(2, E_);                    \
     } while (0)
     switch (epi) {
     case BOX_SPMV_DOT: SPARSH_LAUNCH_BOX1_Q(BOX_SPMV_DOT); break;
@@ -1859,6 +1947,7 @@
     default: SPARSH_LAUNCH_BOX1_Q(BOX_JACOBI_PROLONG); break;
     }
 #undef SPARSH_LAUNCH_BOX1_Q
+#undef SPARSH_LAUNCH_BOX1_BS
 #undef SPARSH_LAUNCH_BOX1
     return nwg;
 }
@@ -1880,21 +1969,28 @@
     for (int u = 0; u < 7; ++u) g.c[u] = A.sd_tab.cval[u];
     g.omega = omega;
     const int chunks = (g.nz + g.CZ - 1) / g.CZ;
-    const dim3 grid(g.ytiles * chunks), block(kBoxBlock);
+    const dim3 grid(g.ytiles * chunks), block(A.box_bs);
     const size_t lds = box2_lds_bytes(g.nx, g.TY);
-#define SPARSH_LAUNCH_BOX(Q_)                                                                                       \
-    do {                                                                                                            \
-        if (from_zero) {                                                                                            \
-            if (finest) hipLaunchKernelGGL((sdia_box2_kernel<Q_, 1, true>), grid, block, lds, st, g, x, b, y);      \
-            else hipLaunchKernelGGL((sdia_box2_kernel<Q_, 0, true>), grid, block, lds, st, g, x, b, y);             \
-        } else {                                                                                                    \
-            if (finest) hipLaunchKernelGGL((sdia_box2_kernel<Q_, 1, false>), grid, block, lds, st, g, x, b, y);     \
-            else hipLaunchKernelGGL((sdia_box2_kernel<Q_, 0, false>), grid, block, lds, st, g, x, b, y);            \
-        }                                                                                                           \
+#define SPARSH_LAUNCH_BOX(BS_, Q_)                                                                                       \
+    do {                                                                                                                 \
+        if (from_zero) {                                                                                                 \
+            if (finest) hipLaunchKernelGGL((sdia_box2_kernel<BS_, Q_, 1, true>), grid, block, lds, st, g, x, b, y);      \
+            else hipLaunchKernelGGL((sdia_box2_kernel<BS_, Q_, 0, true>), grid, block, lds, st, g, x, b, y);             \
+        } else {                                                                                                         \
+            if (finest) hipLaunchKernelGGL((sdia_box2_kernel<BS_, Q_, 1, false>), grid, block, lds, st, g, x, b, y);     \
+            else hipLaunchKernelGGL((sdia_box2_kernel<BS_, Q_, 0, false>), grid, block, lds, st, g, x, b, y);            \
+        }                                                                                                                \
     } while (0)
-    if (A.box_q == 4) SPARSH_LAUNCH_BOX(4);
-    else if (A.box_q == 3) SPARSH_LAUNCH_BOX(3);
-    else SPARSH_LAUNCH_BOX(2);
+#define SPARSH_LAUNCH_BOX_BS(Q_)                              \
+    do {                                                      \
+        if (A.box_bs == 256) SPARSH_LAUNCH_BOX(256, Q_);      \
+        else if (A.box_bs == 512) SPARSH_LAUNCH_BOX(512, Q_); \
+        else SPARSH_LAUNCH_BOX(1024, Q_);                     \
+    } while (0)
+    if (A.box_q == 4) SPARSH_LAUNCH_BOX_BS(4);
+    else if (A.box_q == 3) SPARSH_LAUNCH_BOX_BS(3);
+    else SPARSH_LAUNCH_BOX_BS(2);
+#undef SPARSH_LAUNCH_BOX_BS
 #undef SPARSH_LAUNCH_BOX
 }
 
diff --git a/sparsh_amg_amd/csrc/kernels.hpp b/sparsh_amg_amd/csrc/kernels.hpp
--- a/sparsh_amg_amd/csrc/kernels.hpp
+++ b/sparsh_amg_amd/csrc/kernels.hpp
@@ -45,8 +45,10 @@
     bool has_sdia() const { return sd_ptr != nullptr; }
     int box_nx = 0, box_ny = 0, box_nz = 0;
     int box_q = 0, box_ty = 0, box_cz = 0;
+    int box_bs = 1024;
     bool box_on = false;
     int box1_q = 0, box1_ty = 0, box1_cz = 0;
+    int box1_bs = 1024;
     bool box1_on = false;
     int *int_list = nullptr, *bnd_list = nullptr;
     int nint = 0, nbnd = 0;
@@ -130,7 +132,12 @@
 bool box1_plan(DevCsr &A, bool shared_cu = false);
 bool box1_applies(const DevCsr &A, const KernelConfig &cfg);
 int box1_workgroups(const DevCsr &A);
-const char *box_plan_refusal(const DevCsr &A, int kernel, int Q, int TY, int CZ);
+const char *box_plan_refusal(const DevCsr &A, int kernel, int threads, int Q, int TY, int CZ);
+struct BoxPlan {
+    int threads, q, ty, cz;
+};
+constexpr int kBoxCandidates = 12;
+std::vector<BoxPlan> box_plan_candidates(int kernel, int nx, int ny, int nz, int part_cap);
 int launch_box1(const DevCsr &A, int epi, const CsrArgs &a, bool finest, hipStream_t st);
 bool resid_pair_applies(const DevCsr &A, const KernelConfig &cfg);
 void launch_resid_pair(const DevCsr &A, const CsrArgs &a, bool finest, hipStream_t st, const KernelConfig &cfg);
```

New measurement: 705.9 (median of 6 runs). 1.02x the previous value.
